# JeongsooP/RGB-no-more

Hardware: AMD Instinct MI355X
Metric: images/sec JPEG-Ti DCT 512x512 train step (higher is better)
Workload: dtype bf16

## Files before the change

include/rgbnm.h:

```cpp
#ifndef RGBNM_H
#define RGBNM_H
#include <stddef.h>
#include <stdint.h>

#ifdef __cplusplus
extern "C" {
#endif

#define RGBNM_ABI_VERSION 3
#define RGBNM_DT_F32 0
#define RGBNM_DT_BF16 1
#define RGBNM_DT_F16 2
#define RGBNM_DT_I16 2

#define RGBNM_EPI_NONE 0
#define RGBNM_EPI_RES 1
#define RGBNM_EPI_GELU 2
#define RGBNM_EPI_POS 3
#define RGBNM_EPI_DGELU 4
#define RGBNM_EPI_TANH 5
#define RGBNM_EPI_DTANH 6
#define RGBNM_EPI_RES_DROP 7
#define RGBNM_EPI_GELU_DROP 8

int rgbnm_abi_version(void);
int rgbnm_set_option(const char* name, int value);
int rgbnm_get_option(const char* name);
int rgbnm_trace_collect(int tag, double* ms_total, double* flops_total, double* bytes_total, int* count);
int rgbnm_trace_reserve(int n_events);
const char* rgbnm_strerror(int code);

int rgbnm_gemm_nt(int dtype, int epi, const void* A, int lda, const void* W, int ldw, void* C, int ldc,
                  const float* bias, const void* R, int ldr, void* C2, int ldc2, const float* pos, int pos_period,
                  int M, int N, int K, int c_f32, void* stream);

int rgbnm_gemm_nt_drop(int dtype, int epi, const void* A, int lda, const void* W, int ldw, void* C, int ldc,
                       const float* bias, const void* R, int ldr, void* C2, int ldc2, const float* pos, int pos_period,
                       int M, int N, int K, int c_f32, const void* seed, float p, int site, int block, void* stream);
int rgbnm_dropout_apply(int dtype, const void* seed, float p, int site, int block, const void* x, int ldx, void* y, int ldy,
                        int M, int N, void* stream);

size_t rgbnm_gemm_tn_workspace(int M, int No, int Ki);
size_t rgbnm_gemm_tn_workspace_splits(int No, int Ki, int splits);
int rgbnm_gemm_tn(int dtype, const void* dY, int ldy, const void* X, int ldx, float* dW, float* db, int M, int No,
                  int Ki, int perm_heads, int accumulate, void* workspace, size_t workspace_bytes, void* stream);

void rgbnm_gemm_tn_group_begin(void);
int rgbnm_gemm_tn_group_end(void* stream);
void rgbnm_gemm_tn_group_begin_n(int max_jobs);
void rgbnm_gemm_tn_group_begin_id(int max_jobs, unsigned long long id);
void rgbnm_gemm_tn_group_abort(unsigned long long id);

typedef struct rgbnm_linear_desc {
  long long w_off;
  long long b_off;
  long long ws_off;
  long long wst_off;
  long long bperm_off;
  int N, K;
  int perm_heads;
  int add_identity;
  int ldn;
  int pair;
  int chain_kind;
  long long chain_off;
  int bias_mode;
  int _pad2;
  long long b2_off;
} rgbnm_linear_desc;

int rgbnm_prep_weights(int dtype, const rgbnm_linear_desc* descs_dev, int ndesc, const float* master, void* shadow,
                       float* bias_perm, void* stream);
int rgbnm_prep_weights_chain(int dtype, const rgbnm_linear_desc* descs_dev, int ndesc, const float* master, void* shadow,
                             float* bias_perm, void* chain_fwd, void* chain_bwd, int skip_chain_shadows, void* stream);

int rgbnm_layernorm_fwd(int dtype, const void* x, const float* gamma, const float* beta, void* y, float* mean,
                        float* rstd, int M, int E, float eps, void* stream);
size_t rgbnm_layernorm_bwd_workspace(int M, int E);
int rgbnm_layernorm_bwd(int dtype, const void* dy, const void* x, const float* gamma, const float* mean,
                        const float* rstd, const void* dres, void* dx, float* dgamma, float* dbeta, int M, int E,
                        int accumulate, void* workspace, size_t workspace_bytes, void* stream);
int rgbnm_head_pool_fwd(int dtype, const void* x, const float* gamma, const float* beta, void* pooled, float* mean,
                        float* rstd, int B, int N, int E, float eps, void* stream);
int rgbnm_head_pool_bwd(int dtype, const void* dpooled, const void* x, const float* gamma, const float* mean,
                        const float* rstd, void* dx, float* dgamma, float* dbeta, int B, int N, int E, int accumulate,
                        void* workspace, size_t workspace_bytes, void* stream);

int rgbnm_attention_fwd(int dtype, const void* qkv, void* out, float* lse, int B, int N, int heads, float scale,
                        void* stream);
int rgbnm_attention_bwd(int dtype, const void* qkv, const void* out, const void* dout, const float* lse, void* dqkv,
                        int B, int N, int heads, float scale, void* stream);

int rgbnm_subblock_embed(int in_dtype, int out_dtype, const void* y, const void* cbcr, const float* conv16,
                         void* feat, int B, int Hb, int Wb, int transpose_a, void* stream);
int rgbnm_subblock_embed_mix(int in_dtype, int out_dtype, const void* y, const void* cbcr, const float* lam_dev, const float* conv16,
                             void* feat, int B, int Hb, int Wb, int transpose_a, void* stream);

#define RGBNM_OP_IDENTITY 0
#define RGBNM_OP_AUTOCONTRAST 1
#define RGBNM_OP_POSTERIZE 2
#define RGBNM_OP_SOLARIZEADD 3
#define RGBNM_OP_COLOR 4
#define RGBNM_OP_CONTRAST 5
#define RGBNM_OP_BRIGHTNESS 6
#define RGBNM_OP_MIDFREQAUG 7
#define RGBNM_OP_CUTOUT 8
#define RGBNM_OP_TRANSLATEX 9
#define RGBNM_OP_TRANSLATEY 10
#define RGBNM_OP_ROTATE90 11
#define RGBNM_OP_AUTOSATURATION 12
#define RGBNM_OP_GRAYSCALE 13
#define RGBNM_OP_CHROMADROP 14
#define RGBNM_OP_SHARPNESS 15
#define RGBNM_OP_INVERT 16
#define RGBNM_OP_SOLARIZE 17
#define RGBNM_OP_FREQENHANCE 18
#define RGBNM_OP_EQUALIZE 19

typedef struct rgbnm_aug_params {
  int crop_i, crop_j, crop_h, crop_w;
  int flip;
  int op[2];
  float fmag[2];
  int iarg0[2], iarg1[2], iarg2[2];
} rgbnm_aug_params;

size_t rgbnm_dct_augment_workspace(int B);
int rgbnm_dct_augment(const int16_t* Yq, const int16_t* CbCrq, const int16_t* quant, const rgbnm_aug_params* params_dev,
                      const rgbnm_aug_params* params_host, const float* conv16, const float* filters, void* outY,
                      void* outC, int out_dtype, int B, int Hy, int Wy, int Hc, int Wc, int entry_clamp, int nops,
                      void* workspace, size_t workspace_bytes, void* stream);
size_t rgbnm_dct_augment_workspace_ex(int B, int size);
int rgbnm_dct_augment_ex(const int16_t* Yq, const int16_t* CbCrq, const int16_t* quant, const rgbnm_aug_params* params_dev,
                         const rgbnm_aug_params* params_host, const float* conv16, const float* filters, void* outY,
                         void* outC, int out_dtype, int size, int B, int Hy, int Wy, int Hc, int Wc, int entry_clamp,
                         int nops, void* workspace, size_t workspace_bytes, void* stream);

int rgbnm_dct_augment_packed(const int16_t* Ypacked, const int16_t* Cpacked, const long long* y_off, const long long* c_off,
                             const int16_t* quant, const rgbnm_aug_params* params_dev, const rgbnm_aug_params* params_host,
                             const float* conv16, const float* filters, void* outY, void* outC, int out_dtype, int size, int B,
                             int Hy, int Wy, int Hc, int Wc, int entry_clamp, int nops, void* workspace, size_t workspace_bytes,
                             void* stream);

int rgbnm_softxent(int dl_dtype, const float* logits, const float* soft_target, const long long* hard_target,
                   float* loss_rows, float* loss, void* dlogits, int B, int C, float grad_scale, void* stream);
int rgbnm_softxent_loss(const float* logits, const float* soft_target, const long long* hard_target, float* loss_rows,
                        float* row_stats, float* loss, unsigned* ticket, int B, int C, void* stream);
int rgbnm_softxent_grad(int dl_dtype, const float* logits, const float* soft_target, const long long* hard_target,
                        const float* row_stats, const float* gout_dev, void* dlogits, int B, int C, float grad_scale, void* stream);
int rgbnm_softxent_loss_mix(const float* logits, const long long* labels, const float* mix_lam_dev, float* loss_rows,
                            float* row_stats, float* loss, unsigned* ticket, int B, int C, void* stream);
int rgbnm_softxent_grad_mix(int dl_dtype, const float* logits, const long long* labels, const float* mix_lam_dev,
                            const float* row_stats, const float* gout_dev, void* dlogits, int B, int C, float grad_scale,
                            void* stream);
int rgbnm_mixup(int in_dtype, int out_dtype, const void* in, void* out, const float* lam_dev, int B,
                long long per_sample, void* stream);
int rgbnm_mixup_target(const long long* labels, float* target, const float* lam_dev, int B, int C, void* stream);
size_t rgbnm_clip_adamw_wd_workspace(void);
int rgbnm_clip_adamw_wd_step(float* p, const float* g, float* m, float* v, const unsigned char* wd_flag_per_256,
                             long long n, float lr, float beta1, float beta2, float eps, int step, float wd_factor,
                             float max_norm, float* norm_out, void* workspace, size_t workspace_bytes, void* stream);

typedef struct rgbnm_vit_cfg {
  int dtype, B, N, E, heads;
  float ln_eps, attn_scale;
} rgbnm_vit_cfg;

typedef struct rgbnm_block_params {
  const float *ln1_g, *ln1_b, *ln2_g, *ln2_b;
  const float *bqkv_perm, *bproj, *b1, *b2;
  const void *wqkv, *wqkv_t, *wproj, *wproj_t, *w1, *w1_t, *w2, *w2_t;
} rgbnm_block_params;

typedef struct rgbnm_block_acts {
  void* x_in;
  void* xn1;
  float *mean1, *rstd1;
  void* qkv;
  float* lse;
  void* attn;
  void* x_mid;
  void* xn2;
  float *mean2, *rstd2;
  void* u;
  void* gl;
  void* x_out;
} rgbnm_block_acts;

typedef struct rgbnm_block_grads {
  float *dln1_g, *dln1_b, *dln2_g, *dln2_b;
  float *dwqkv, *dbqkv, *dwproj, *dbproj, *dw1, *db1, *dw2, *db2;
} rgbnm_block_grads;

typedef struct rgbnm_block_scratch {
  void* du;
  void* dxn;
  void* dx_mid;
  void* dattn;
  void* dqkv;
  void* ws;
  size_t ws_bytes;
} rgbnm_block_scratch;

size_t rgbnm_vit_workspace(const rgbnm_vit_cfg* cfg);
size_t rgbnm_vit_workspace_ex(const rgbnm_vit_cfg* cfg, int n_classes);
int rgbnm_vit_block_fwd(const rgbnm_vit_cfg* cfg, const rgbnm_block_params* p, const rgbnm_block_acts* a,
                        void* stream);
int rgbnm_vit_ln_chain(const rgbnm_vit_cfg* cfg);
int rgbnm_vit_block_fwd_chain(const rgbnm_vit_cfg* cfg, const rgbnm_block_params* p, const rgbnm_block_acts* a,
                              int flags, const rgbnm_block_params* next_p, const rgbnm_block_acts* next_a,
                              void* stream);
int rgbnm_vit_block_bwd(const rgbnm_vit_cfg* cfg, const rgbnm_block_params* p, const rgbnm_block_acts* a,
                        const rgbnm_block_grads* g, const rgbnm_block_scratch* s, const void* dy, void* dx,
                        void* stream);

typedef struct rgbnm_dropout {
  const void* seed;
  float p;
  int block;
  void *dy_m, *dxmid_m;
} rgbnm_dropout;
int rgbnm_vit_block_fwd_drop(const rgbnm_vit_cfg* cfg, const rgbnm_block_params* p, const rgbnm_block_acts* a,
                             const rgbnm_dropout* d, void* stream);
int rgbnm_vit_block_bwd_drop(const rgbnm_vit_cfg* cfg, const rgbnm_block_params* p, const rgbnm_block_acts* a,
                             const rgbnm_block_grads* g, const rgbnm_block_scratch* s, const rgbnm_dropout* d, const void* dy,
                             void* dx, void* stream);

typedef struct rgbnm_chain_block {
  const void* wimg;
  const float *ln1_g, *ln1_b, *ln2_g, *ln2_b, *bqkv_perm, *bproj, *b1, *b2;
  void* xn1; float *mean1, *rstd1;
  void* qkv; float* lse; void* attn; void* x_mid; void* xn2; float *mean2, *rstd2;
  void* u; void* gl; void* x_out;
} rgbnm_chain_block;
size_t rgbnm_chain_block_bytes(void);
long long rgbnm_chain_image_elems(void);
int rgbnm_chain_gather(const void* src, const int* idx, void* dst, long long n, void* stream);
int rgbnm_vit_chain_fwd(const rgbnm_vit_cfg* cfg, const rgbnm_chain_block* blocks, int depth, const void* x0, void* stream);

typedef struct rgbnm_chain_bwd_block {
  const void* wimg;
  const float *ln1_g, *ln2_g;
  const void* x_in; const float *mean1, *rstd1;
  const void* qkv; const float* lse; const void* attn; const void* x_mid; const float *mean2, *rstd2; const void* u;
  const void* dy;
  void* du; void* dx_mid; void* dqkv; void* dx;
  float *part2, *part1;
} rgbnm_chain_bwd_block;
size_t rgbnm_chain_bwd_block_bytes(void);
int rgbnm_vit_chain_bwd(const rgbnm_vit_cfg* cfg, const rgbnm_chain_bwd_block* blocks, int depth, void* dattn, void* stream);
int rgbnm_vit_block_bwd_dw(const rgbnm_vit_cfg* cfg, const rgbnm_block_acts* a, const rgbnm_block_grads* g,
                           const rgbnm_block_scratch* s, const void* dy, const float* part2, const float* part1, void* stream);
int rgbnm_vit_blocks_bwd_dw(const rgbnm_vit_cfg* cfg, int n, const rgbnm_block_acts* const* a, const rgbnm_block_grads* const* g,
                            const rgbnm_block_scratch* const* s, const void* const* dy, const float* const* part2,
                            const float* const* part1, void* stream);
int rgbnm_vit_blocks_bwd_dw_pe(const rgbnm_vit_cfg* cfg, int n, const rgbnm_block_acts* const* a, const rgbnm_block_grads* const* g,
                               const rgbnm_block_scratch* const* s, const void* const* dy, const float* const* part2,
                               const float* const* part1, const void* pe_dx0, const void* pe_feat, float* pe_dw, float* pe_db,
                               void* pe_ws, size_t pe_ws_bytes, void* stream);

int rgbnm_gelu_table_init(void* stream);
int rgbnm_gelu_table_info(int* win16, unsigned* full65536);

int rgbnm_reduce_hold_begin(void);
int rgbnm_reduce_hold_end(void* table, void* table_host, size_t table_bytes, void* stream);
void rgbnm_reduce_hold_cancel(void);
size_t rgbnm_reduce_hold_table_bytes(void);

int rgbnm_patch_embed_fwd(const rgbnm_vit_cfg* cfg, int in_dtype, const void* y, const void* cbcr,
                          const float* conv16, const void* wpe, const float* bpe, const float* pos, void* feat,
                          void* x0, int Hb, int Wb, void* stream);
int rgbnm_patch_embed_fwd_mix(const rgbnm_vit_cfg* cfg, int in_dtype, const void* y, const void* cbcr, const float* lam_dev,
                              const float* conv16, const void* wpe, const float* bpe, const float* pos, void* feat, void* x0,
                              int Hb, int Wb, void* stream);
int rgbnm_patch_embed_bwd(const rgbnm_vit_cfg* cfg, const void* dx0, const void* feat, float* dwpe, float* dbpe,
                          void* ws, size_t ws_bytes, void* stream);

typedef struct rgbnm_head_params {
  const float *ln_g, *ln_b, *b1, *b2;
  const void *w1, *w1_t, *w2, *w2_t;
  int n_classes;
  int _pad;
} rgbnm_head_params;
typedef struct rgbnm_head_acts {
  void* x;
  float *mean, *rstd;
  void* pooled;
  void* h1;
  float* logits;
} rgbnm_head_acts;
typedef struct rgbnm_head_grads {
  float *dln_g, *dln_b, *dw1, *db1, *dw2, *db2;
} rgbnm_head_grads;
int rgbnm_head_fwd(const rgbnm_vit_cfg* cfg, const rgbnm_head_params* p, const rgbnm_head_acts* a, void* stream);
size_t rgbnm_head_bwd_workspace(const rgbnm_vit_cfg* cfg, int n_classes);
int rgbnm_head_bwd(const rgbnm_vit_cfg* cfg, const rgbnm_head_params* p, const rgbnm_head_acts* a,
                   const rgbnm_head_grads* g, const void* dlogits, void* da, void* dpooled, void* dx, void* ws,
                   size_t ws_bytes, void* stream);

int rgbnm_swin_embed(int in_dtype, int out_dtype, const void* y, const void* cbcr, const float* convY, const float* convC,
                     void* feat, int B, int Hb, int Wb, void* stream);
int rgbnm_ln_generic_fwd(int dtype, const void* x, const float* gamma, const float* beta, const void* res,
                         const float* sample_scale, int rows_per_sample, void* y, float* mean, float* rstd, int M, int E,
                         float eps, void* stream);
size_t rgbnm_ln_generic_bwd_workspace(int M, int E);
int rgbnm_ln_generic_bwd(int dtype, const void* dy, const void* x, const float* gamma, const float* mean,
                         const float* rstd, const float* sample_scale, int rows_per_sample, void* dx, float* dgamma,
                         float* dbeta, int M, int E, int accumulate, void* workspace, size_t workspace_bytes,
                         void* stream);
int rgbnm_window_attention_fwd(int dtype, const void* qkv, const float* bias, const float* scale, void* out, float* lse,
                               int B, int res, int C, int heads, int shift, void* stream);
size_t rgbnm_window_attention_bwd_workspace(int B, int res, int heads);
int rgbnm_window_attention_bwd(int dtype, const void* qkv, const void* out, const void* dout, const float* bias,
                               float* dscale , const float* scale, const float* lse, void* dqkv,
                               float* dbias, float* dscale_part, int B, int res, int C, int heads, int shift, void* workspace,
                               size_t workspace_bytes, void* stream);
typedef struct rgbnm_cpb_block {
  const float *w1, *b1, *w2, *ls;
  float *bias, *scale;
  const float *dbias, *dscale;
  float *dw1, *db1, *dw2, *dls;
  int heads, _pad;
} rgbnm_cpb_block;
size_t rgbnm_swin_cpb_table_elems(int nblocks);
int rgbnm_swin_cpb_fwd(const rgbnm_cpb_block* blocks, int nblocks, const float* coords, const int* index, float* table, void* stream);
int rgbnm_swin_cpb_bwd(const rgbnm_cpb_block* blocks, int nblocks, const float* coords, const int* inv_index, const float* table,
                       float* dtable, void* stream);
int rgbnm_merge_gather(int dtype, const void* in, void* out, int B, int res, int C, int inverse, void* stream);
int rgbnm_token_mean(int dtype, const void* in, void* out, int B, int N, int C, int backward, void* stream);


int rgbnm_calib_mfma_bf16(int workgroups, int iters, float* sink, void* stream);
int rgbnm_calib_stream(const void* src, void* dst, size_t bytes, int mode, int workgroups, void* sink, void* stream);
int rgbnm_calib_vmem_issue(int mode, int workgroups, int waves, void* buf, size_t wave_bytes, int ld,
                           unsigned long long* out, void* stream);
int rgbnm_calib_l2(const void* buf, size_t slice_bytes, int iters, int mode, int workgroups, int waves, void* sink,
                   void* stream);
int rgbnm_calib_pipes(const int* role_dev, int waves, int iters, int workgroups, unsigned long long* out, float* sink,
                      void* stream);

int rgbnm_calib_occupy(const void* buf, size_t slice_bytes, int workgroups, int lds_bytes, long long ticks, int mode,
                       const int* stop, void* sink, void* stream);
int rgbnm_calib_occupy_log(const void* buf, size_t slice_bytes, int workgroups, int lds_bytes, long long ticks, int mode,
                           const int* stop, void* sink, unsigned long long* log, void* stream);

#ifdef __cplusplus
}
#endif
#endif
```

rgb-no-more_amd/csrc/gemm_nt_small.hip:

```cpp
#include "common.h"
#include "internal.h"

namespace {

enum { EPI_NONE = 0, EPI_TANH = 5, EPI_DTANH = 6 };

struct SmallNT {
  const bf16* A; const bf16* W; void* C; const float* bias; const bf16* R;
  int lda, ldw, ldc, ldr;
  int M, N, K, c_f32, ntiles;
};

constexpr int RP = 36;

template <int EPI>
__global__ __launch_bounds__(256) void gemm_nt_small_kernel(SmallNT p) {
  __shared__ __attribute__((aligned(16))) float red[4][32 * RP];
  const int tid = threadIdx.x, lane = tid & 63;
  const int w = __builtin_amdgcn_readfirstlane(tid >> 6);
  const int l31 = lane & 31, g = lane >> 5;
  const int m0 = (blockIdx.x / p.ntiles) * 32, n0 = (blockIdx.x % p.ntiles) * 32;
  const bf16* arow = p.A + (size_t)min(m0 + l31, p.M - 1) * p.lda;
  const bf16* wrow = p.W + (size_t)min(n0 + l31, p.N - 1) * p.ldw;
  const int ksteps = (p.K + 15) / 16;
  const int per = (ksteps + 3) / 4;
  const int s0 = w * per, s1 = min(s0 + per, ksteps);
  f32x16 acc;
#pragma unroll
  for (int r = 0; r < 16; ++r) acc[r] = 0.f;
  const bf16x8 zero = {0, 0, 0, 0, 0, 0, 0, 0};
  auto frag = [&](const bf16* row, int s) -> bf16x8 {
    const int k = 16 * s + 8 * g;
    return k < p.K ? *reinterpret_cast<const bf16x8*>(row + k) : zero;
  };
  for (int s = s0; s < s1; s += 4) {
    Frag<bf16> fa[4], fw[4];
#pragma unroll
    for (int u = 0; u < 4; ++u) {
      const int su = s + u < s1 ? s + u : s1 - 1;
      fa[u].v = frag(arow, su);
      fw[u].v = frag(wrow, su);
    }
#pragma unroll
    for (int u = 0; u < 4; ++u)
      if (s + u < s1) mma(acc, fw[u], fa[u]);
  }
#pragma unroll
  for (int q = 0; q < 4; ++q) {
    const f32x4 v = {acc[4 * q + 0], acc[4 * q + 1], acc[4 * q + 2], acc[4 * q + 3]};
    *reinterpret_cast<f32x4*>(&red[w][l31 * RP + 8 * q + 4 * g]) = v;
  }
  __syncthreads();
  const int row = tid >> 3, f0 = (tid & 7) * 4;
  const int gm = m0 + row, gn = n0 + f0;
  if (gm >= p.M || gn >= p.N) return;
  f32x4 v = *reinterpret_cast<const f32x4*>(&red[0][row * RP + f0]);
#pragma unroll
  for (int k = 1; k < 4; ++k) v += *reinterpret_cast<const f32x4*>(&red[k][row * RP + f0]);
  if (p.bias) v += *reinterpret_cast<const f32x4*>(p.bias + gn);
  if (p.c_f32) {
#pragma unroll
    for (int e = 0; e < 4; ++e) {
      if (EPI == EPI_TANH) v[e] = tanhf(v[e]);
      if (EPI == EPI_DTANH) {
        const float h = (float)p.R[(size_t)gm * p.ldr + gn + e];
        v[e] *= (1.f - h * h);
      }
    }
    *reinterpret_cast<f32x4*>(reinterpret_cast<float*>(p.C) + (size_t)gm * p.ldc + gn) = v;
    return;
  }
  bf16x4 o;
#pragma unroll
  for (int e = 0; e < 4; ++e) {
    float x = (float)(bf16)v[e];
    if (EPI == EPI_TANH) x = tanhf(x);
    if (EPI == EPI_DTANH) {
      const float h = (float)p.R[(size_t)gm * p.ldr + gn + e];
      x *= (1.f - h * h);
    }
    o[e] = (bf16)x;
  }
  *reinterpret_cast<bf16x4*>(reinterpret_cast<bf16*>(p.C) + (size_t)gm * p.ldc + gn) = o;
}

}

int rgbnm_launch_nt_small(int epi, const void* A, int lda, const void* W, int ldw, void* C, int ldc, const float* bias,
                          const void* R, int ldr, int c_f32, int M, int N, int K, hipStream_t st) {
  if (M > 512 || K % 8 || N % 4 || lda % 8 || ldw % 8 || ldc % 4 || (epi != EPI_NONE && epi != EPI_TANH && epi != EPI_DTANH))
    return 1;
  if (epi == EPI_DTANH && !R) return RGBNM_EINVAL;
  SmallNT p;
  p.A = (const bf16*)A; p.W = (const bf16*)W; p.C = C; p.bias = bias; p.R = (const bf16*)R;
  p.lda = lda; p.ldw = ldw; p.ldc = ldc; p.ldr = ldr; p.M = M; p.N = N; p.K = K; p.c_f32 = c_f32;
  p.ntiles = cdiv(N, 32);
  const int grid = cdiv(M, 32) * p.ntiles;
  const double mn = (double)M * N;
  const int slot = rgbnm_trace_begin(TR_NT, 2.0 * mn * K, ((double)M * K + (double)N * K) * 2.0 + mn * (c_f32 ? 4.0 : 2.0) +
                                                              (epi == EPI_DTANH ? mn * 2.0 : 0.0), st);
  switch (epi) {
    case EPI_NONE: hipLaunchKernelGGL(gemm_nt_small_kernel<EPI_NONE>, dim3(grid), dim3(256), 0, st, p); break;
    case EPI_TANH: hipLaunchKernelGGL(gemm_nt_small_kernel<EPI_TANH>, dim3(grid), dim3(256), 0, st, p); break;
    default: hipLaunchKernelGGL(gemm_nt_small_kernel<EPI_DTANH>, dim3(grid), dim3(256), 0, st, p); break;
  }
  rgbnm_trace_end(slot, st);
  LAUNCH_CHECK();
  return RGBNM_OK;
}
```

rgb-no-more_amd/csrc/internal.h:

```cpp
#pragma once
#include <hip/hip_runtime.h>

constexpr int RGBNM_TN_MAX_SPLIT = 128;
struct RgbnmTnJob {
  const void* dY; const void* X; float* part; float* bpart;
  int ldy, ldx, M, No, Ki;
  float* dW; float* db; int perm_heads, accumulate;
  int smax;
};
int rgbnm_launch_tn_pipe_group(const RgbnmTnJob* jobs, int n, int* S_out, hipStream_t st, int* direct_out = nullptr);
void rgbnm_tn_defer_begin();
void rgbnm_tn_defer_begin_n(int max_jobs);
int rgbnm_tn_defer_flush(hipStream_t st);
int rgbnm_launch_tn_pipe(const void* dY, int ldy, const void* X, int ldx, float* part, float* bpart, int M, int No,
                         int Ki, int* S_out, hipStream_t st, int smax = 0);

int rgbnm_launch_attn2_fwd(const void* qkv, void* out, float* lse, int B, int N, int heads, float scale,
                           hipStream_t st);
int rgbnm_launch_attn2_bwd(const void* qkv, const void* out, const void* dout, const float* lse, void* dqkv, int B,
                           int N, int heads, float scale, hipStream_t st);

enum { TR_NT = 1, TR_TN = 2, TR_ATTN_FWD = 3, TR_ATTN_BWD = 4, TR_CHAIN_FWD = 5, TR_CHAIN_BWD = 6, TR_AUG = 7, TR_EMBED = 8, TR_OPT = 9 };
int rgbnm_launch_nt_wres(int epi, const void* A, int lda, const void* W, int ldw, void* C, int ldc, const float* bias,
                         const void* R, int ldr, void* C2, int ldc2, int M, int N, int K, hipStream_t st);
int rgbnm_launch_nt_kpipe(int epi, const void* A, int lda, const void* W, int ldw, void* C, int ldc, const float* bias,
                          const void* R, int ldr, void* C2, int ldc2, int M, int N, int K, hipStream_t st);
int rgbnm_launch_nt_kpipe_res_ln(const void* A, int lda, const void* W, int ldw, const float* bias, const void* R,
                                 int ldr, void* x, int ldc, const float* gamma, const float* beta, void* y, int ldy,
                                 float* mean, float* rstd, float eps, int M, int N, int K, hipStream_t st);
int rgbnm_launch_mlp_fwd(const void* X, int ldx, const void* W1, const float* b1, const void* W2, const float* b2,
                         const void* R, int ldr, void* G, void* GP, int ldg, void* Y, int ldy, const float* gamma,
                         const float* beta, void* Y2, int ldy2, float* mean, float* rstd, float eps, int M, int E, int H,
                         hipStream_t st);
int rgbnm_launch_nt_small(int epi, const void* A, int lda, const void* W, int ldw, void* C, int ldc, const float* bias,
                          const void* R, int ldr, int c_f32, int M, int N, int K, hipStream_t st);
int rgbnm_launch_mlp_bwd(const void* DY, int lddy, const void* W2T, const void* W1T, const void* GP, int ldg, void* DU, int ldu,
                         const void* X, int ldx, const float* gamma, const float* mean, const float* rstd, void* DX, int lddx,
                         float* part, int* npanels_out, int M, int E, int H, hipStream_t st);
int rgbnm_launch_nt_kpipe_lnbwd(const void* A, int lda, const void* W, int ldw, const void* X, int ldx,
                                const float* gamma, const float* mean, const float* rstd, const void* dres, int ldr,
                                void* dx, int ldc, float* part, int* npanels_out, int M, int N, int K, hipStream_t st);
struct RgbnmReduceJob {
  const float* part; long long stride; float* out;
  int n, S, cols, perm_heads, accumulate, epw;
};
bool rgbnm_reduce_defer_active();
void rgbnm_reduce_defer_begin();
int rgbnm_reduce_defer_flush(hipStream_t st);
int rgbnm_reduce_submit(const RgbnmReduceJob& job, hipStream_t st);
int rgbnm_trace_begin(int tag, double flops, double bytes, hipStream_t st);
void rgbnm_trace_end(int slot, hipStream_t st);
```

rgb-no-more_amd/csrc/reduce.hip:

```cpp
#include <cstddef>
#include <cstring>
#include "common.h"
#include "internal.h"

namespace {

constexpr int MAXJOBS = 16;
struct Jobs {
  RgbnmReduceJob j[MAXJOBS];
};

thread_local bool g_defer = false;
thread_local int g_njobs = 0;
thread_local Jobs g_jobs;

__device__ __forceinline__ int qkv_row_r(int n, int heads) {
  const int inner = heads * 64;
  const int s3 = n / inner, rem = n % inner;
  return (rem / 64) * 192 + (rem % 64) * 3 + s3;
}

__global__ __launch_bounds__(256) void reduce_multi_kernel(Jobs J) {
  const RgbnmReduceJob jb = J.j[blockIdx.y];
  __shared__ float red[256];
  const int epw = jb.epw, nsg = 256 / epw;
  const int el = threadIdx.x % epw, sg = threadIdx.x / epw;
  for (int base = blockIdx.x * epw; base < jb.n; base += gridDim.x * epw) {
    const int i = base + el;
    float a = 0.f;
    if (i < jb.n) {
      const float* src = jb.part + i;
#pragma unroll 8
      for (int s = sg; s < jb.S; s += nsg) a += src[(size_t)s * jb.stride];
    }
    red[sg * epw + el] = a;
    __syncthreads();
    if (sg == 0 && i < jb.n) {
      float t;
      if (nsg == 4) {
        t = (red[el] + red[epw + el]) + (red[2 * epw + el] + red[3 * epw + el]);
      } else {
        t = 0.f;
        for (int g = 0; g < nsg; ++g) t += red[g * epw + el];
      }
      int o = i;
      if (jb.perm_heads > 0) {
        const int r = i / jb.cols, c = i % jb.cols;
        o = qkv_row_r(r, jb.perm_heads) * jb.cols + c;
      }
      jb.out[o] = jb.accumulate ? (jb.out[o] + t) : t;
    }
    __syncthreads();
  }
}

constexpr int MAXHELD = 384;
struct HeldTable {
  int njobs, total;
  int first[MAXHELD + 1];
  unsigned char vec[MAXHELD];
  RgbnmReduceJob j[MAXHELD];
};
thread_local bool g_hold = false;
thread_local HeldTable g_held;

template <int VEC>
__device__ __forceinline__ void reduce_job(const RgbnmReduceJob& jb, int bx, int nbx, float* red) {
  const int epw = jb.epw, nsg = 256 / epw;
  const int el = threadIdx.x % epw, sg = threadIdx.x / epw;
  for (int base = bx * epw * VEC; base < jb.n; base += nbx * epw * VEC) {
    const int i = base + el * VEC;
    float a[VEC];
#pragma unroll
    for (int v = 0; v < VEC; ++v) a[v] = 0.f;
    if (i < jb.n) {
      const float* src = jb.part + i;
#pragma unroll 8
      for (int s = sg; s < jb.S; s += nsg) {
        if (VEC == 4) {
          const f32x4 q = *reinterpret_cast<const f32x4*>(src + (size_t)s * jb.stride);
#pragma unroll
          for (int v = 0; v < VEC; ++v) a[v] += q[v];
        } else {
          a[0] += src[(size_t)s * jb.stride];
        }
      }
    }
#pragma unroll
    for (int v = 0; v < VEC; ++v) red[(sg * epw + el) * VEC + v] = a[v];
    __syncthreads();
    if (sg == 0 && i < jb.n) {
#pragma unroll
      for (int v = 0; v < VEC; ++v) {
        float t;
        if (nsg == 4) {
          t = (red[el * VEC + v] + red[(epw + el) * VEC + v]) + (red[(2 * epw + el) * VEC + v] + red[(3 * epw + el) * VEC + v]);
        } else {
          t = 0.f;
          for (int g = 0; g < nsg; ++g) t += red[(g * epw + el) * VEC + v];
        }
        int o = i + v;
        if (jb.perm_heads > 0) {
          const int r = o / jb.cols, c = o % jb.cols;
          o = qkv_row_r(r, jb.perm_heads) * jb.cols + c;
        }
        jb.out[o] = jb.accumulate ? (jb.out[o] + t) : t;
      }
    }
    __syncthreads();
  }
}

__global__ __launch_bounds__(256) void reduce_table_kernel(const HeldTable* __restrict__ T) {
  __shared__ __attribute__((aligned(16))) float red[256 * 4];
  int lo = 0, hi = T->njobs - 1;
  while (lo < hi) {
    const int mid = (lo + hi + 1) >> 1;
    if (T->first[mid] <= (int)blockIdx.x) lo = mid;
    else hi = mid - 1;
  }
  const RgbnmReduceJob jb = T->j[lo];
  const int bx = blockIdx.x - T->first[lo], nbx = T->first[lo + 1] - T->first[lo];
  if (T->vec[lo]) reduce_job<4>(jb, bx, nbx, red);
  else reduce_job<1>(jb, bx, nbx, red);
}

int launch(const Jobs& J, int njobs, hipStream_t st) {
  int gx = 1;
  for (int k = 0; k < njobs; ++k) {
    const int need = cdiv(J.j[k].n, J.j[k].epw);
    gx = need > gx ? need : gx;
  }
  if (gx > 1024) gx = 1024;
  hipLaunchKernelGGL(reduce_multi_kernel, dim3(gx, njobs), dim3(256), 0, st, J);
  LAUNCH_CHECK();
  return RGBNM_OK;
}

}

bool rgbnm_reduce_defer_active() { return g_defer; }
void rgbnm_reduce_defer_begin() {
  g_defer = true;
  g_njobs = 0;
}

int rgbnm_reduce_defer_flush(hipStream_t st) {
  g_defer = false;
  const int n = g_njobs;
  g_njobs = 0;
  return n > 0 ? launch(g_jobs, n, st) : RGBNM_OK;
}

int rgbnm_reduce_submit(const RgbnmReduceJob& job, hipStream_t st) {
  if (job.n <= 0 || job.S <= 0 || (job.epw != 64 && job.epw != 8)) return RGBNM_EINVAL;
  if (g_hold && g_held.njobs < MAXHELD) {
    g_held.j[g_held.njobs++] = job;
    return RGBNM_OK;
  }
  if (g_defer) {
    if (g_njobs == MAXJOBS) {
      const int rc = launch(g_jobs, g_njobs, st);
      if (rc != RGBNM_OK) return rc;
      g_njobs = 0;
    }
    g_jobs.j[g_njobs++] = job;
    return RGBNM_OK;
  }
  Jobs one;
  one.j[0] = job;
  return launch(one, 1, st);
}

extern "C" {

int rgbnm_reduce_hold_begin(void) {
  if (g_hold) return RGBNM_EINVAL;
  g_hold = true;
  g_held.njobs = 0;
  return RGBNM_OK;
}

void rgbnm_reduce_hold_cancel(void) {
  g_hold = false;
  g_held.njobs = 0;
}

int rgbnm_reduce_hold_end(void* table_dev, void* table_host, size_t table_bytes, void* stream) {
  if (!g_hold) return RGBNM_OK;
  g_hold = false;
  const int n = g_held.njobs;
  if (n == 0) return RGBNM_OK;
  if (!table_dev || !table_host || table_bytes < sizeof(HeldTable)) return RGBNM_EWORKSPACE;
  int total = 0;
  for (int k = 0; k < n; ++k) {
    const RgbnmReduceJob& j = g_held.j[k];
    const bool vec = j.n % 4 == 0 && j.stride % 4 == 0 && ((size_t)j.part & 15) == 0 && (j.perm_heads <= 0 || j.cols % 4 == 0);
    g_held.vec[k] = vec ? 1 : 0;
    g_held.first[k] = total;
    const int need = cdiv(j.n, j.epw * (vec ? 4 : 1));
    total += need > 1024 ? 1024 : need;
  }
  for (int k = n; k <= MAXHELD; ++k) g_held.first[k] = total;
  g_held.total = total;
  hipStream_t st = (hipStream_t)stream;
  const size_t used = offsetof(HeldTable, j) + sizeof(RgbnmReduceJob) * (size_t)n;
  if (memcmp(table_host, &g_held, used) != 0) {
    hipStreamCaptureStatus cap = hipStreamCaptureStatusNone;
    if (hipStreamIsCapturing(st, &cap) != hipSuccess) { g_held.njobs = 0; return RGBNM_ELAUNCH; }
    if (cap != hipStreamCaptureStatusNone) {
      memcpy(table_host, &g_held, used);
      if (hipMemcpyAsync(table_dev, table_host, used, hipMemcpyHostToDevice, st) != hipSuccess) {
        (void)hipGetLastError();
        memset(table_host, 0, used);
        g_held.njobs = 0;
        return RGBNM_EINVAL;
      }
    } else {
      if (hipMemcpyAsync(table_dev, &g_held, used, hipMemcpyHostToDevice, st) != hipSuccess) {
        g_held.njobs = 0;
        return RGBNM_ELAUNCH;
      }
      memcpy(table_host, &g_held, used);
    }
  }
  g_held.njobs = 0;
  hipLaunchKernelGGL(reduce_table_kernel, dim3(total), dim3(256), 0, st, (const HeldTable*)table_dev);
  LAUNCH_CHECK();
  return RGBNM_OK;
}

size_t rgbnm_reduce_hold_table_bytes(void) { return sizeof(HeldTable); }

}
```

rgb-no-more_amd/csrc/vit.hip:

```cpp
#include "common.h"
#include "../../include/rgbnm.h"

#define TRY(x)                 \
  do {                         \
    int rc__ = (x);            \
    if (rc__ != 0) return rc__; \
  } while (0)

static inline size_t max_sz(size_t a, size_t b) { return a > b ? a : b; }

#include <string.h>
#include <atomic>
#include <mutex>
#include <vector>
#include "internal.h"
namespace {
std::mutex g_trace_mu;
struct TraceRec { hipEvent_t a, b; int tag; double flops, bytes; };
std::vector<TraceRec> g_recs;
std::vector<hipEvent_t> g_event_pool;
hipEvent_t take_event() {
  if (!g_event_pool.empty()) { hipEvent_t e = g_event_pool.back(); g_event_pool.pop_back(); return e; }
  hipEvent_t e = nullptr;
  if (hipEventCreate(&e) != hipSuccess) return nullptr;
  return e;
}
struct Opt { const char* name; std::atomic<int> value; };
Opt g_opts[] = {{"nt_staged", 1}, {"tn_tr", 1}, {"tn_pipe", 1}, {"attn_v2", 1}, {"nt_wres", 1}, {"nt_kpipe", 1}, {"attn_persist", 1}, {"ln_fuse", 1}, {"tn_group", 2}, {"trace", 0}, {"tn_wgs", 512}, {"mlp_fuse", 1}, {"nt_cold", 0}, {"mlp_bwd", 1}, {"nt_small", 1}, {"mlp_dmast", 1}, {"gelu_table", 1}, {"ln_rows", 1}, {"kp8", 1}, {"win_xcd", 1}, {"kp_persist", 1}, {"fwd_chain", 1}, {"bwd_chain", 1}, {"tn_direct", 1}, {"tn_pack", 1}, {"tn_wide", 1}};
}

int rgbnm_trace_begin(int tag, double flops, double bytes, hipStream_t st) {
  int mask = 0;
  for (auto& o : g_opts) if (!strcmp(o.name, "trace")) mask = o.value.load(std::memory_order_relaxed);
  if (!((mask >> tag) & 1)) return -1;
  std::lock_guard<std::mutex> lk(g_trace_mu);
  TraceRec r;
  r.a = take_event();
  r.b = take_event();
  if (!r.a || !r.b) return -1;
  r.tag = tag; r.flops = flops; r.bytes = bytes;
  (void)hipEventRecord(r.a, st);
  g_recs.push_back(r);
  return (int)g_recs.size() - 1;
}
void rgbnm_trace_end(int slot, hipStream_t st) {
  if (slot < 0) return;
  std::lock_guard<std::mutex> lk(g_trace_mu);
  if (slot >= 0 && slot < (int)g_recs.size()) (void)hipEventRecord(g_recs[slot].b, st);
}

extern "C" {

int rgbnm_abi_version(void) { return RGBNM_ABI_VERSION; }

int rgbnm_set_option(const char* name, int value) {
  for (auto& o : g_opts)
    if (name && !strcmp(o.name, name)) { o.value.store(value, std::memory_order_relaxed); return RGBNM_OK; }
  return RGBNM_EINVAL;
}
int rgbnm_get_option(const char* name) {
  for (auto& o : g_opts)
    if (name && !strcmp(o.name, name)) return o.value.load(std::memory_order_relaxed);
  return -1;
}

int rgbnm_trace_reserve(int n_events) {
  if (n_events < 0 || n_events > (1 << 16)) return RGBNM_EINVAL;
  std::lock_guard<std::mutex> lk(g_trace_mu);
  while ((int)g_event_pool.size() < n_events) {
    hipEvent_t e = nullptr;
    if (hipEventCreate(&e) != hipSuccess) return RGBNM_ELAUNCH;
    g_event_pool.push_back(e);
  }
  return RGBNM_OK;
}

int rgbnm_trace_collect(int tag, double* ms_total, double* flops_total, double* bytes_total, int* count) {
  double ms = 0, fl = 0, by = 0;
  int n = 0;
  std::lock_guard<std::mutex> lk(g_trace_mu);
  std::vector<TraceRec> keep;
  for (auto& r : g_recs) {
    if (r.tag != tag) { keep.push_back(r); continue; }
    if (hipEventSynchronize(r.b) != hipSuccess) return RGBNM_ELAUNCH;
    float t = 0.f;
    if (hipEventElapsedTime(&t, r.a, r.b) != hipSuccess) return RGBNM_ELAUNCH;
    ms += t; fl += r.flops; by += r.bytes; ++n;
    g_event_pool.push_back(r.a);
    g_event_pool.push_back(r.b);
  }
  g_recs.swap(keep);
  if (ms_total) *ms_total = ms;
  if (flops_total) *flops_total = fl;
  if (bytes_total) *bytes_total = by;
  if (count) *count = n;
  return RGBNM_OK;
}

const char* rgbnm_strerror(int code) {
  switch (code) {
    case 0: return "ok";
    case RGBNM_EINVAL: return "invalid argument (null pointer, bad shape, alignment or dtype)";
    case RGBNM_ELAUNCH: return "HIP kernel launch failed";
    case RGBNM_EWORKSPACE: return "workspace too small";
    default: return "unknown rgbnm error";
  }
}

static bool fused_dx_lnbwd(int dt, const void* A, int lda, const void* Wt, int ldw, const void* x, const float* gamma,
                           const float* mean, const float* rstd, const void* dres, void* dx, float* dgamma,
                           float* dbeta, int M, int E, int K, void* ws, size_t ws_bytes, hipStream_t st) {
  if (dt != RGBNM_DT_BF16 || E != 192 || !rgbnm_get_option("ln_fuse") || !rgbnm_get_option("nt_kpipe")) return false;
  if (ws_bytes < (size_t)cdiv(M, cdiv(M, 512)) * 2 * E * sizeof(float)) return false;
  int npanels = 0;
  const int rc = rgbnm_launch_nt_kpipe_lnbwd(A, lda, Wt, ldw, x, E, gamma, mean, rstd, dres, E, dx, E, (float*)ws,
                                             &npanels, M, E, K, st);
  if (rc != RGBNM_OK) return false;
  RgbnmReduceJob j;
  j.part = (const float*)ws; j.stride = 2LL * E; j.out = dgamma; j.n = E; j.S = npanels; j.cols = 1; j.perm_heads = 0;
  j.accumulate = 0; j.epw = 8;
  if (rgbnm_reduce_submit(j, st) != RGBNM_OK) return false;
  j.part = (const float*)ws + E; j.out = dbeta;
  return rgbnm_reduce_submit(j, st) == RGBNM_OK;
}

static bool fused_mlp_bwd(int dt, const void* dy, const void* w2t, const void* w1t, const void* gp, void* du, const void* x,
                          const float* gamma, const float* mean, const float* rstd, void* dx, float* dgamma, float* dbeta,
                          int M, int E, void* ws, size_t ws_bytes, hipStream_t st) {
  if (dt != RGBNM_DT_BF16 || E != 192 || !rgbnm_get_option("mlp_bwd") || !rgbnm_get_option("ln_fuse")) return false;
  if (ws_bytes < (size_t)cdiv(M, cdiv(M, 256)) * 2 * E * sizeof(float)) return false;
  int npanels = 0;
  const int rc = rgbnm_launch_mlp_bwd(dy, E, w2t, w1t, gp, 4 * E, du, 4 * E, x, E, gamma, mean, rstd, dx, E, (float*)ws,
                                      &npanels, M, E, 4 * E, st);
  if (rc != RGBNM_OK) return false;
  RgbnmReduceJob j;
  j.part = (const float*)ws; j.stride = 2LL * E; j.out = dgamma; j.n = E; j.S = npanels; j.cols = 1; j.perm_heads = 0;
  j.accumulate = 0; j.epw = 8;
  if (rgbnm_reduce_submit(j, st) != RGBNM_OK) return false;
  j.part = (const float*)ws + E; j.out = dbeta;
  return rgbnm_reduce_submit(j, st) == RGBNM_OK;
}

static size_t block_ws_offsets(int M, int E, int I, size_t (&off)[7]) {
  const size_t sz[6] = {rgbnm_gemm_tn_workspace(M, E, 4 * E), rgbnm_gemm_tn_workspace(M, 4 * E, E),
                        rgbnm_gemm_tn_workspace(M, E, I),     rgbnm_gemm_tn_workspace(M, 3 * I, E),
                        rgbnm_layernorm_bwd_workspace(M, E),  rgbnm_layernorm_bwd_workspace(M, E)};
  off[0] = 0;
  for (int i = 0; i < 6; ++i) off[i + 1] = off[i] + ((sz[i] + 255) & ~(size_t)255);
  return off[6];
}

size_t rgbnm_vit_workspace(const rgbnm_vit_cfg* c) { return rgbnm_vit_workspace_ex(c, 1024); }

size_t rgbnm_vit_workspace_ex(const rgbnm_vit_cfg* c, int n_classes) {
  if (!c) return 0;
  if (n_classes < 1024) n_classes = 1024;
  const int M = c->B * c->N, E = c->E, I = c->heads * 64;
  size_t off[7];
  size_t w = block_ws_offsets(M, E, I, off);
  w = max_sz(w, rgbnm_gemm_tn_workspace(M, E, 384));
  w = max_sz(w, rgbnm_gemm_tn_workspace(c->B, n_classes, E));
  w = max_sz(w, rgbnm_layernorm_bwd_workspace(M, E));
  w = max_sz(w, (size_t)c->B * 2 * E * sizeof(float));
  return w;
}

int rgbnm_vit_ln_chain(const rgbnm_vit_cfg* c) {
  if (!c) return 0;
  return c->dtype == RGBNM_DT_BF16 && c->E == 192 && c->B * c->N >= 8192 && rgbnm_get_option("ln_fuse") &&
         rgbnm_get_option("nt_kpipe");
}

int rgbnm_vit_block_fwd_chain(const rgbnm_vit_cfg* c, const rgbnm_block_params* p, const rgbnm_block_acts* a, int flags,
                              const rgbnm_block_params* next_p, const rgbnm_block_acts* next_a, void* st) {
  if (!c || !p || !a) return RGBNM_EINVAL;
  const int dt = c->dtype, M = c->B * c->N, E = c->E, I = c->heads * 64;
  const bool chain = rgbnm_vit_ln_chain(c) != 0;
  if ((flags & 1) && !chain) return RGBNM_EINVAL;
  if (!(flags & 1))
    TRY(rgbnm_layernorm_fwd(dt, a->x_in, p->ln1_g, p->ln1_b, a->xn1, a->mean1, a->rstd1, M, E, c->ln_eps, st));
  TRY(rgbnm_gemm_nt(dt, RGBNM_EPI_NONE, a->xn1, E, p->wqkv, E, a->qkv, 3 * I, p->bqkv_perm, 0, 0, 0, 0, 0, 0, M,
                    3 * I, E, 0, st));
  TRY(rgbnm_attention_fwd(dt, a->qkv, a->attn, a->lse, c->B, c->N, c->heads, c->attn_scale, st));
  if (!chain || rgbnm_launch_nt_kpipe_res_ln(a->attn, I, p->wproj, I, p->bproj, a->x_in, E, a->x_mid, E, p->ln2_g,
                                             p->ln2_b, a->xn2, E, a->mean2, a->rstd2, c->ln_eps, M, E, I,
                                             (hipStream_t)st) != RGBNM_OK) {
    TRY(rgbnm_gemm_nt(dt, RGBNM_EPI_RES, a->attn, I, p->wproj, I, a->x_mid, E, p->bproj, a->x_in, E, 0, 0, 0, 0, M, E,
                      I, 0, st));
    TRY(rgbnm_layernorm_fwd(dt, a->x_mid, p->ln2_g, p->ln2_b, a->xn2, a->mean2, a->rstd2, M, E, c->ln_eps, st));
  }
  const bool to_next = chain && next_p && next_a;
  if (to_next && next_a->x_in != a->x_out) return RGBNM_EINVAL;
  if (dt == RGBNM_DT_BF16 && rgbnm_get_option("mlp_fuse")) {
    const int rc = rgbnm_launch_mlp_fwd(a->xn2, E, p->w1, p->b1, p->w2, p->b2, a->x_mid, E, a->gl, a->u, 4 * E, a->x_out, E,
                                        to_next ? next_p->ln1_g : nullptr, to_next ? next_p->ln1_b : nullptr,
                                        to_next ? next_a->xn1 : nullptr, E, to_next ? next_a->mean1 : nullptr,
                                        to_next ? next_a->rstd1 : nullptr, c->ln_eps, M, E, 4 * E, (hipStream_t)st);
    if (rc <= 0) return rc;
  }
  TRY(rgbnm_gemm_nt(dt, RGBNM_EPI_GELU, a->xn2, E, p->w1, E, a->gl, 4 * E, p->b1, 0, 0, a->u, 4 * E, 0, 0, M, 4 * E,
                    E, 0, st));
  if (to_next) {
    const int rc = rgbnm_launch_nt_kpipe_res_ln(a->gl, 4 * E, p->w2, 4 * E, p->b2, a->x_mid, E, a->x_out, E,
                                                next_p->ln1_g, next_p->ln1_b, next_a->xn1, E, next_a->mean1,
                                                next_a->rstd1, c->ln_eps, M, E, 4 * E, (hipStream_t)st);
    if (rc != RGBNM_OK) return rc < 0 ? rc : RGBNM_EINVAL;
    return RGBNM_OK;
  }
  TRY(rgbnm_gemm_nt(dt, RGBNM_EPI_RES, a->gl, 4 * E, p->w2, 4 * E, a->x_out, E, p->b2, a->x_mid, E, 0, 0, 0, 0, M, E,
                    4 * E, 0, st));
  return RGBNM_OK;
}

int rgbnm_vit_block_fwd(const rgbnm_vit_cfg* c, const rgbnm_block_params* p, const rgbnm_block_acts* a, void* st) {
  return rgbnm_vit_block_fwd_chain(c, p, a, 0, nullptr, nullptr, st);
}

int rgbnm_vit_block_fwd_drop(const rgbnm_vit_cfg* c, const rgbnm_block_params* p, const rgbnm_block_acts* a, const rgbnm_dropout* d,
                             void* st) {
  if (!c || !p || !a || !d) return RGBNM_EINVAL;
  const int dt = c->dtype, M = c->B * c->N, E = c->E, I = c->heads * 64;
  TRY(rgbnm_layernorm_fwd(dt, a->x_in, p->ln1_g, p->ln1_b, a->xn1, a->mean1, a->rstd1, M, E, c->ln_eps, st));
  TRY(rgbnm_gemm_nt(dt, RGBNM_EPI_NONE, a->xn1, E, p->wqkv, E, a->qkv, 3 * I, p->bqkv_perm, 0, 0, 0, 0, 0, 0, M,
                    3 * I, E, 0, st));
  TRY(rgbnm_attention_fwd(dt, a->qkv, a->attn, a->lse, c->B, c->N, c->heads, c->attn_scale, st));
  TRY(rgbnm_gemm_nt_drop(dt, RGBNM_EPI_RES_DROP, a->attn, I, p->wproj, I, a->x_mid, E, p->bproj, a->x_in, E, 0, 0, 0, 0, M, E, I,
                         0, d->seed, d->p, 0, d->block, st));
  TRY(rgbnm_layernorm_fwd(dt, a->x_mid, p->ln2_g, p->ln2_b, a->xn2, a->mean2, a->rstd2, M, E, c->ln_eps, st));
  TRY(rgbnm_gemm_nt_drop(dt, RGBNM_EPI_GELU_DROP, a->xn2, E, p->w1, E, a->gl, 4 * E, p->b1, 0, 0, a->u, 4 * E, 0, 0, M, 4 * E, E,
                         0, d->seed, d->p, 1, d->block, st));
  TRY(rgbnm_gemm_nt_drop(dt, RGBNM_EPI_RES_DROP, a->gl, 4 * E, p->w2, 4 * E, a->x_out, E, p->b2, a->x_mid, E, 0, 0, 0, 0, M, E,
                         4 * E, 0, d->seed, d->p, 2, d->block, st));
  return RGBNM_OK;
}

static int block_bwd(const rgbnm_vit_cfg* c, const rgbnm_block_params* p, const rgbnm_block_acts* a, const rgbnm_block_grads* g,
                     const rgbnm_block_scratch* s, const rgbnm_dropout* d, const void* dy, void* dx, void* st) {
  if (!c || !p || !a || !g || !s || !dy || !dx) return RGBNM_EINVAL;
  if (d && (!d->dy_m || !d->dxmid_m || d->dy_m == d->dxmid_m)) return RGBNM_EINVAL;
  const int dt = c->dtype, M = c->B * c->N, E = c->E, I = c->heads * 64;
  size_t off[7];
  if (s->ws_bytes < block_ws_offsets(M, E, I, off)) return RGBNM_EWORKSPACE;
  char* wsb = (char*)s->ws;
#define WS(i) (wsb + off[i]), (off[(i) + 1] - off[i])
  rgbnm_reduce_defer_begin();
  bool tn_open = false;
  const int rc = [&]() -> int {
  int group = rgbnm_get_option("tn_group");
  const bool wide4 = rgbnm_get_option("tn_wide") && E % 384 == 0 && I % 384 == 0 && M % 64 == 0;
  if (group == 2 && E > 192 && !wide4) group = 1;
  if (group) { rgbnm_tn_defer_begin(); tn_open = true; }
  const void* dyg = dy;
  if (d) {
    TRY(rgbnm_dropout_apply(dt, d->seed, d->p, 2, d->block, dy, E, d->dy_m, E, M, E, st));
    dyg = d->dy_m;
  }
  TRY(rgbnm_gemm_tn(dt, dyg, E, a->gl, 4 * E, g->dw2, g->db2, M, E, 4 * E, 0, 0, WS(0), st));
  const bool mlp_bwd_fused = !d && fused_mlp_bwd(dt, dy, p->w2_t, p->w1_t, a->u, s->du, a->x_mid, p->ln2_g, a->mean2, a->rstd2,
                                                 s->dx_mid, g->dln2_g, g->dln2_b, M, E, WS(4), (hipStream_t)st);
  if (!mlp_bwd_fused)
    TRY(rgbnm_gemm_nt(dt, RGBNM_EPI_DGELU, dyg, E, p->w2_t, E, s->du, 4 * E, 0, a->u, 4 * E, 0, 0, 0, 0, M, 4 * E, E, 0,
                      st));
  TRY(rgbnm_gemm_tn(dt, s->du, 4 * E, a->xn2, E, g->dw1, g->db1, M, 4 * E, E, 0, 0, WS(1), st));
  if (group == 1) { tn_open = false; TRY(rgbnm_tn_defer_flush((hipStream_t)st)); }
  if (mlp_bwd_fused) {
  } else if (!fused_dx_lnbwd(dt, s->du, 4 * E, p->w1_t, 4 * E, a->x_mid, p->ln2_g, a->mean2, a->rstd2, dy, s->dx_mid,
                      g->dln2_g, g->dln2_b, M, E, 4 * E, WS(4), (hipStream_t)st)) {
    TRY(rgbnm_gemm_nt(dt, RGBNM_EPI_NONE, s->du, 4 * E, p->w1_t, 4 * E, s->dxn, E, 0, 0, 0, 0, 0, 0, 0, M, E, 4 * E,
                      0, st));
    TRY(rgbnm_layernorm_bwd(dt, s->dxn, a->x_mid, p->ln2_g, a->mean2, a->rstd2, dy, s->dx_mid, g->dln2_g, g->dln2_b,
                            M, E, 0, WS(4), st));
  }
  const void* dxmg = s->dx_mid;
  if (d) {
    TRY(rgbnm_dropout_apply(dt, d->seed, d->p, 0, d->block, s->dx_mid, E, d->dxmid_m, E, M, E, st));
    dxmg = d->dxmid_m;
  }
  if (group == 1) { rgbnm_tn_defer_begin(); tn_open = true; }
  TRY(rgbnm_gemm_tn(dt, dxmg, E, a->attn, I, g->dwproj, g->dbproj, M, E, I, 0, 0, WS(2), st));
  TRY(rgbnm_gemm_nt(dt, RGBNM_EPI_NONE, dxmg, E, p->wproj_t, E, s->dattn, I, 0, 0, 0, 0, 0, 0, 0, M, I, E, 0, st));
  TRY(rgbnm_attention_bwd(dt, a->qkv, a->attn, s->dattn, a->lse, s->dqkv, c->B, c->N, c->heads, c->attn_scale, st));
  TRY(rgbnm_gemm_tn(dt, s->dqkv, 3 * I, a->xn1, E, g->dwqkv, g->dbqkv, M, 3 * I, E, c->heads, 0, WS(3), st));
  if (group) { tn_open = false; TRY(rgbnm_tn_defer_flush((hipStream_t)st)); }
  if (!fused_dx_lnbwd(dt, s->dqkv, 3 * I, p->wqkv_t, 3 * I, a->x_in, p->ln1_g, a->mean1, a->rstd1, s->dx_mid, dx,
                      g->dln1_g, g->dln1_b, M, E, 3 * I, WS(5), (hipStream_t)st)) {
    TRY(rgbnm_gemm_nt(dt, RGBNM_EPI_NONE, s->dqkv, 3 * I, p->wqkv_t, 3 * I, s->dxn, E, 0, 0, 0, 0, 0, 0, 0, M, E,
                      3 * I, 0, st));
    TRY(rgbnm_layernorm_bwd(dt, s->dxn, a->x_in, p->ln1_g, a->mean1, a->rstd1, s->dx_mid, dx, g->dln1_g, g->dln1_b, M,
                            E, 0, WS(5), st));
  }
  return RGBNM_OK;
  }();
#undef WS
  const int rt = tn_open ? rgbnm_tn_defer_flush((hipStream_t)st) : RGBNM_OK;
  const int rf = rgbnm_reduce_defer_flush((hipStream_t)st);
  return rc != RGBNM_OK ? rc : (rt != RGBNM_OK ? rt : rf);
}

int rgbnm_vit_block_bwd(const rgbnm_vit_cfg* c, const rgbnm_block_params* p, const rgbnm_block_acts* a,
                        const rgbnm_block_grads* g, const rgbnm_block_scratch* s, const void* dy, void* dx, void* st) {
  return block_bwd(c, p, a, g, s, nullptr, dy, dx, st);
}

int rgbnm_vit_block_bwd_drop(const rgbnm_vit_cfg* c, const rgbnm_block_params* p, const rgbnm_block_acts* a,
                             const rgbnm_block_grads* g, const rgbnm_block_scratch* s, const rgbnm_dropout* d, const void* dy,
                             void* dx, void* st) {
  if (!d) return RGBNM_EINVAL;
  return block_bwd(c, p, a, g, s, d, dy, dx, st);
}

int rgbnm_vit_blocks_bwd_dw(const rgbnm_vit_cfg* c, int n, const rgbnm_block_acts* const* a, const rgbnm_block_grads* const* g,
                            const rgbnm_block_scratch* const* s, const void* const* dy, const float* const* part2,
                            const float* const* part1, void* st) {
  return rgbnm_vit_blocks_bwd_dw_pe(c, n, a, g, s, dy, part2, part1, nullptr, nullptr, nullptr, nullptr, nullptr, 0, st);
}

int rgbnm_vit_blocks_bwd_dw_pe(const rgbnm_vit_cfg* c, int n, const rgbnm_block_acts* const* a, const rgbnm_block_grads* const* g,
                               const rgbnm_block_scratch* const* s, const void* const* dy, const float* const* part2,
                               const float* const* part1, const void* pe_dx0, const void* pe_feat, float* pe_dw, float* pe_db,
                               void* pe_ws, size_t pe_ws_bytes, void* st) {
  if (!c || n < 1 || n > 12 || !a || !g || !s || !dy || !part2 || !part1) return RGBNM_EINVAL;
  if (pe_dx0 && (!pe_feat || !pe_dw || !pe_ws)) return RGBNM_EINVAL;
  const int dt = c->dtype, M = c->B * c->N, E = c->E, I = c->heads * 64;
  size_t off[7];
  const size_t need = block_ws_offsets(M, E, I, off);
  for (int i = 0; i < n; ++i) {
    if (!a[i] || !g[i] || !s[i] || !dy[i] || !part2[i] || !part1[i]) return RGBNM_EINVAL;
    if (s[i]->ws_bytes < need) return RGBNM_EWORKSPACE;
    for (int k = 0; k < i; ++k)
      if (s[k]->ws == s[i]->ws) return RGBNM_EINVAL;
  }
  rgbnm_reduce_defer_begin();
  bool tn_open = false;
  const int rc = [&]() -> int {
    const int group = rgbnm_get_option("tn_group");
    if (group) { rgbnm_tn_defer_begin_n(group == 1 ? 2 : 4 * n + (pe_dx0 ? 1 : 0)); tn_open = true; }
    for (int i = 0; i < n; ++i) {
      char* wsb = (char*)s[i]->ws;
#define WS(k) (wsb + off[k]), (off[(k) + 1] - off[k])
      TRY(rgbnm_gemm_tn(dt, dy[i], E, a[i]->gl, 4 * E, g[i]->dw2, g[i]->db2, M, E, 4 * E, 0, 0, WS(0), st));
      TRY(rgbnm_gemm_tn(dt, s[i]->du, 4 * E, a[i]->xn2, E, g[i]->dw1, g[i]->db1, M, 4 * E, E, 0, 0, WS(1), st));
      TRY(rgbnm_gemm_tn(dt, s[i]->dx_mid, E, a[i]->attn, I, g[i]->dwproj, g[i]->dbproj, M, E, I, 0, 0, WS(2), st));
      TRY(rgbnm_gemm_tn(dt, s[i]->dqkv, 3 * I, a[i]->xn1, E, g[i]->dwqkv, g[i]->dbqkv, M, 3 * I, E, c->heads, 0, WS(3), st));
#undef WS
    }
    if (pe_dx0) TRY(rgbnm_gemm_tn(dt, pe_dx0, E, pe_feat, 384, pe_dw, pe_db, M, E, 384, 0, 0, pe_ws, pe_ws_bytes, st));
    if (group) { tn_open = false; TRY(rgbnm_tn_defer_flush((hipStream_t)st)); }
    for (int i = 0; i < n; ++i) {
      RgbnmReduceJob j;
      j.stride = 2LL * E; j.n = E; j.S = c->B; j.cols = 1; j.perm_heads = 0; j.accumulate = 0; j.epw = 8;
      j.part = part2[i]; j.out = g[i]->dln2_g;
      TRY(rgbnm_reduce_submit(j, (hipStream_t)st));
      j.part = part2[i] + E; j.out = g[i]->dln2_b;
      TRY(rgbnm_reduce_submit(j, (hipStream_t)st));
      j.part = part1[i]; j.out = g[i]->dln1_g;
      TRY(rgbnm_reduce_submit(j, (hipStream_t)st));
      j.part = part1[i] + E; j.out = g[i]->dln1_b;
      TRY(rgbnm_reduce_submit(j, (hipStream_t)st));
    }
    return RGBNM_OK;
  }();
  const int rt = tn_open ? rgbnm_tn_defer_flush((hipStream_t)st) : RGBNM_OK;
  const int rf = rgbnm_reduce_defer_flush((hipStream_t)st);
  return rc != RGBNM_OK ? rc : (rt != RGBNM_OK ? rt : rf);
}

int rgbnm_vit_block_bwd_dw(const rgbnm_vit_cfg* c, const rgbnm_block_acts* a, const rgbnm_block_grads* g,
                           const rgbnm_block_scratch* s, const void* dy, const float* part2, const float* part1, void* st) {
  return rgbnm_vit_blocks_bwd_dw(c, 1, &a, &g, &s, &dy, &part2, &part1, st);
}

int rgbnm_patch_embed_fwd_mix(const rgbnm_vit_cfg* c, int in_dtype, const void* y, const void* cbcr, const float* lam_dev,
                              const float* conv16, const void* wpe, const float* bpe, const float* pos, void* feat, void* x0, int Hb,
                              int Wb, void* st) {
  if (!c) return RGBNM_EINVAL;
  const int M = c->B * c->N;
  if ((Hb / 2) * (Wb / 2) != c->N) return RGBNM_EINVAL;
  TRY(rgbnm_subblock_embed_mix(in_dtype, c->dtype, y, cbcr, lam_dev, conv16, feat, c->B, Hb, Wb, 0, st));
  TRY(rgbnm_gemm_nt(c->dtype, RGBNM_EPI_POS, feat, 384, wpe, 384, x0, c->E, bpe, 0, 0, 0, 0, pos, c->N, M, c->E, 384,
                    0, st));
  return RGBNM_OK;
}

int rgbnm_patch_embed_fwd(const rgbnm_vit_cfg* c, int in_dtype, const void* y, const void* cbcr, const float* conv16,
                          const void* wpe, const float* bpe, const float* pos, void* feat, void* x0, int Hb, int Wb,
                          void* st) {
  return rgbnm_patch_embed_fwd_mix(c, in_dtype, y, cbcr, nullptr, conv16, wpe, bpe, pos, feat, x0, Hb, Wb, st);
}

int rgbnm_patch_embed_bwd(const rgbnm_vit_cfg* c, const void* dx0, const void* feat, float* dwpe, float* dbpe,
                          void* ws, size_t ws_bytes, void* st) {
  if (!c) return RGBNM_EINVAL;
  return rgbnm_gemm_tn(c->dtype, dx0, c->E, feat, 384, dwpe, dbpe, c->B * c->N, c->E, 384, 0, 0, ws, ws_bytes, st);
}

int rgbnm_head_fwd(const rgbnm_vit_cfg* c, const rgbnm_head_params* p, const rgbnm_head_acts* a, void* st) {
  if (!c || !p || !a) return RGBNM_EINVAL;
  const int dt = c->dtype, E = c->E, C = p->n_classes;
  TRY(rgbnm_head_pool_fwd(dt, a->x, p->ln_g, p->ln_b, a->pooled, a->mean, a->rstd, c->B, c->N, E, c->ln_eps, st));
  TRY(rgbnm_gemm_nt(dt, RGBNM_EPI_TANH, a->pooled, E, p->w1, E, a->h1, E, p->b1, 0, 0, 0, 0, 0, 0, c->B, E, E, 0, st));
  TRY(rgbnm_gemm_nt(dt, RGBNM_EPI_NONE, a->h1, E, p->w2, E, a->logits, C, p->b2, 0, 0, 0, 0, 0, 0, c->B, C, E, 1, st));
  return RGBNM_OK;
}

size_t rgbnm_head_bwd_workspace(const rgbnm_vit_cfg* c, int n_classes) {
  if (!c) return 0;
  return ((rgbnm_gemm_tn_workspace(c->B, n_classes, c->E) + 255) & ~(size_t)255) + ((rgbnm_gemm_tn_workspace(c->B, c->E, c->E) + 255) & ~(size_t)255) +
         (size_t)c->B * 2 * c->E * sizeof(float);
}

int rgbnm_head_bwd(const rgbnm_vit_cfg* c, const rgbnm_head_params* p, const rgbnm_head_acts* a,
                   const rgbnm_head_grads* g, const void* dlogits, void* da, void* dpooled, void* dx, void* ws,
                   size_t ws_bytes, void* st) {
  if (!c || !p || !a || !g || !dlogits || !da || !dpooled || !dx) return RGBNM_EINVAL;
  const int dt = c->dtype, E = c->E, C = p->n_classes, B = c->B;
  const size_t s1 = (rgbnm_gemm_tn_workspace(B, C, E) + 255) & ~(size_t)255, s2 = (rgbnm_gemm_tn_workspace(B, E, E) + 255) & ~(size_t)255;
  const size_t s3 = (size_t)B * 2 * E * sizeof(float);
  const bool apart = ws_bytes >= s1 + s2 + s3;
  char* w1 = (char*)ws;
  char* w2 = apart ? w1 + s1 : w1;
  char* w3 = apart ? w2 + s2 : w1;
  const size_t b1 = apart ? s1 : ws_bytes, b2 = apart ? s2 : ws_bytes, b3 = apart ? ws_bytes - s1 - s2 : ws_bytes;
  const bool grouped = apart && rgbnm_get_option("tn_group") != 0;
  if (grouped) rgbnm_tn_defer_begin();
  const int rc = [&]() -> int {
    TRY(rgbnm_gemm_tn(dt, dlogits, C, a->h1, E, g->dw2, g->db2, B, C, E, 0, 0, w1, b1, st));
    TRY(rgbnm_gemm_nt(dt, RGBNM_EPI_DTANH, dlogits, C, p->w2_t, C, da, E, 0, a->h1, E, 0, 0, 0, 0, B, E, C, 0, st));
    TRY(rgbnm_gemm_tn(dt, da, E, a->pooled, E, g->dw1, g->db1, B, E, E, 0, 0, w2, b2, st));
    return RGBNM_OK;
  }();
  const int rt = grouped ? rgbnm_tn_defer_flush((hipStream_t)st) : RGBNM_OK;
  if (rc != RGBNM_OK) return rc;
  if (rt != RGBNM_OK) return rt;
  TRY(rgbnm_gemm_nt(dt, RGBNM_EPI_NONE, da, E, p->w1_t, E, dpooled, E, 0, 0, 0, 0, 0, 0, 0, B, E, E, 0, st));
  TRY(rgbnm_head_pool_bwd(dt, dpooled, a->x, p->ln_g, a->mean, a->rstd, dx, g->dln_g, g->dln_b, B, c->N, E, 0, w3, b3, st));
  return RGBNM_OK;
}

}
```

rgb-no-more_amd/lib.py:

```python
import ctypes as C
import os

import torch

HERE = os.path.dirname(os.path.abspath(__file__))
LIB_PATH = os.path.join(HERE, "librgbnm.so")

DT_F32, DT_BF16, DT_F16 = 0, 1, 2
EPI_NONE, EPI_RES, EPI_GELU, EPI_POS, EPI_DGELU, EPI_TANH, EPI_DTANH = range(7)
EPI_RES_DROP, EPI_GELU_DROP = 7, 8

_vp, _i, _f, _sz, _ll = C.c_void_p, C.c_int, C.c_float, C.c_size_t, C.c_longlong
HOST_WAIT = {"sec": 0.0}


class LinearDesc(C.Structure):
    _fields_ = [("w_off", _ll), ("b_off", _ll), ("ws_off", _ll), ("wst_off", _ll), ("bperm_off", _ll),
                ("N", _i), ("K", _i), ("perm_heads", _i), ("add_identity", _i), ("ldn", _i), ("pair", _i),
                ("chain_kind", _i), ("chain_off", _ll), ("bias_mode", _i), ("_pad2", _i), ("b2_off", _ll)]


class VitCfg(C.Structure):
    _fields_ = [("dtype", _i), ("B", _i), ("N", _i), ("E", _i), ("heads", _i), ("ln_eps", _f), ("attn_scale", _f)]


class BlockParams(C.Structure):
    _fields_ = [(n, _vp) for n in ("ln1_g", "ln1_b", "ln2_g", "ln2_b", "bqkv_perm", "bproj", "b1", "b2",
                                   "wqkv", "wqkv_t", "wproj", "wproj_t", "w1", "w1_t", "w2", "w2_t")]


class BlockActs(C.Structure):
    _fields_ = [(n, _vp) for n in ("x_in", "xn1", "mean1", "rstd1", "qkv", "lse", "attn", "x_mid", "xn2", "mean2",
                                   "rstd2", "u", "gl", "x_out")]


class BlockGrads(C.Structure):
    _fields_ = [(n, _vp) for n in ("dln1_g", "dln1_b", "dln2_g", "dln2_b", "dwqkv", "dbqkv", "dwproj", "dbproj",
                                   "dw1", "db1", "dw2", "db2")]


class BlockScratch(C.Structure):
    _fields_ = [("du", _vp), ("dxn", _vp), ("dx_mid", _vp), ("dattn", _vp), ("dqkv", _vp), ("ws", _vp),
                ("ws_bytes", _sz)]


class Dropout(C.Structure):
    _fields_ = [("seed", _vp), ("p", _f), ("block", _i), ("dy_m", _vp), ("dxmid_m", _vp)]


class HeadParams(C.Structure):
    _fields_ = [(n, _vp) for n in ("ln_g", "ln_b", "b1", "b2", "w1", "w1_t", "w2", "w2_t")] + \
               [("n_classes", _i), ("_pad", _i)]


class HeadActs(C.Structure):
    _fields_ = [(n, _vp) for n in ("x", "mean", "rstd", "pooled", "h1", "logits")]


class HeadGrads(C.Structure):
    _fields_ = [(n, _vp) for n in ("dln_g", "dln_b", "dw1", "db1", "dw2", "db2")]


class CpbBlock(C.Structure):
    _fields_ = [(n, _vp) for n in ("w1", "b1", "w2", "ls", "bias", "scale", "dbias", "dscale", "dw1", "db1", "dw2", "dls")] + \
               [("heads", _i), ("_pad", _i)]


class ChainBlock(C.Structure):
    _fields_ = [(n, _vp) for n in ("wimg", "ln1_g", "ln1_b", "ln2_g", "ln2_b", "bqkv_perm", "bproj", "b1", "b2", "xn1", "mean1",
                                   "rstd1", "qkv", "lse", "attn", "x_mid", "xn2", "mean2", "rstd2", "u", "gl", "x_out")]


class ChainBwdBlock(C.Structure):
    _fields_ = [(n, _vp) for n in ("wimg", "ln1_g", "ln2_g", "x_in", "mean1", "rstd1", "qkv", "lse", "attn", "x_mid", "mean2",
                                   "rstd2", "u", "dy", "du", "dx_mid", "dqkv", "dx", "part2", "part1")]


ABI_VERSION = 3

_P = C.POINTER
PROTOTYPES = {
    "rgbnm_abi_version": (_i, []),
    "rgbnm_strerror": (C.c_char_p, [_i]),
    "rgbnm_set_option": (_i, [C.c_char_p, _i]),
    "rgbnm_gemm_tn_group_begin": (None, []),
    "rgbnm_gemm_tn_group_begin_n": (None, [_i]),
    "rgbnm_gemm_tn_group_begin_id": (None, [_i, C.c_ulonglong]),
    "rgbnm_gemm_tn_group_abort": (None, [C.c_ulonglong]),
    "rgbnm_gemm_tn_group_end": (_i, [_vp]),
    "rgbnm_get_option": (_i, [C.c_char_p]),
    "rgbnm_trace_collect": (_i, [_i, _vp, _vp, _vp, _vp]),
    "rgbnm_trace_reserve": (_i, [_i]),
    "rgbnm_gemm_nt": (_i, [_i, _i, _vp, _i, _vp, _i, _vp, _i, _vp, _vp, _i, _vp, _i, _vp, _i, _i, _i, _i, _i, _vp]),
    "rgbnm_gemm_nt_drop": (_i, [_i, _i, _vp, _i, _vp, _i, _vp, _i, _vp, _vp, _i, _vp, _i, _vp, _i, _i, _i, _i, _i, _vp, _f, _i,
                                _i, _vp]),
    "rgbnm_dropout_apply": (_i, [_i, _vp, _f, _i, _i, _vp, _i, _vp, _i, _i, _i, _vp]),
    "rgbnm_gemm_tn_workspace": (_sz, [_i, _i, _i]),
    "rgbnm_gemm_tn_workspace_splits": (_sz, [_i, _i, _i]),
    "rgbnm_gemm_tn": (_i, [_i, _vp, _i, _vp, _i, _vp, _vp, _i, _i, _i, _i, _i, _vp, _sz, _vp]),
    "rgbnm_prep_weights": (_i, [_i, _vp, _i, _vp, _vp, _vp, _vp]),
    "rgbnm_prep_weights_chain": (_i, [_i, _vp, _i, _vp, _vp, _vp, _vp, _vp, _i, _vp]),
    "rgbnm_layernorm_fwd": (_i, [_i, _vp, _vp, _vp, _vp, _vp, _vp, _i, _i, _f, _vp]),
    "rgbnm_layernorm_bwd_workspace": (_sz, [_i, _i]),
    "rgbnm_layernorm_bwd": (_i, [_i, _vp, _vp, _vp, _vp, _vp, _vp, _vp, _vp, _vp, _i, _i, _i, _vp, _sz, _vp]),
    "rgbnm_head_pool_fwd": (_i, [_i, _vp, _vp, _vp, _vp, _vp, _vp, _i, _i, _i, _f, _vp]),
    "rgbnm_head_pool_bwd": (_i, [_i, _vp, _vp, _vp, _vp, _vp, _vp, _vp, _vp, _i, _i, _i, _i, _vp, _sz, _vp]),
    "rgbnm_attention_fwd": (_i, [_i, _vp, _vp, _vp, _i, _i, _i, _f, _vp]),
    "rgbnm_attention_bwd": (_i, [_i, _vp, _vp, _vp, _vp, _vp, _i, _i, _i, _f, _vp]),
    "rgbnm_subblock_embed": (_i, [_i, _i, _vp, _vp, _vp, _vp, _i, _i, _i, _i, _vp]),
    "rgbnm_subblock_embed_mix": (_i, [_i, _i, _vp, _vp, _vp, _vp, _vp, _i, _i, _i, _i, _vp]),
    "rgbnm_dct_augment_workspace": (_sz, [_i]),
    "rgbnm_dct_augment": (_i, [_vp, _vp, _vp, _vp, _vp, _vp, _vp, _vp, _vp, _i, _i, _i, _i, _i, _i, _i, _i, _vp, _sz,
                               _vp]),
    "rgbnm_dct_augment_workspace_ex": (_sz, [_i, _i]),
    "rgbnm_dct_augment_ex": (_i, [_vp, _vp, _vp, _vp, _vp, _vp, _vp, _vp, _vp, _i, _i, _i, _i, _i, _i, _i, _i, _i, _vp,
                                  _sz, _vp]),
    "rgbnm_dct_augment_packed": (_i, [_vp, _vp, _vp, _vp, _vp, _vp, _vp, _vp, _vp, _vp, _vp, _i, _i, _i, _i, _i, _i, _i, _i,
                                      _i, _vp, _sz, _vp]),
    "rgbnm_softxent": (_i, [_i, _vp, _vp, _vp, _vp, _vp, _vp, _i, _i, _f, _vp]),
    "rgbnm_softxent_loss": (_i, [_vp, _vp, _vp, _vp, _vp, _vp, _vp, _i, _i, _vp]),
    "rgbnm_softxent_grad": (_i, [_i, _vp, _vp, _vp, _vp, _vp, _vp, _i, _i, _f, _vp]),
    "rgbnm_softxent_loss_mix": (_i, [_vp, _vp, _vp, _vp, _vp, _vp, _vp, _i, _i, _vp]),
    "rgbnm_softxent_grad_mix": (_i, [_i, _vp, _vp, _vp, _vp, _vp, _vp, _i, _i, _f, _vp]),
    "rgbnm_mixup": (_i, [_i, _i, _vp, _vp, _vp, _i, _ll, _vp]),
    "rgbnm_mixup_target": (_i, [_vp, _vp, _vp, _i, _i, _vp]),
    "rgbnm_clip_adamw_wd_workspace": (_sz, []),
    "rgbnm_clip_adamw_wd_step": (_i, [_vp, _vp, _vp, _vp, _vp, _ll, _f, _f, _f, _f, _i, _f, _f, _vp, _vp, _sz, _vp]),
    "rgbnm_vit_workspace": (_sz, [_P(VitCfg)]),
    "rgbnm_vit_workspace_ex": (_sz, [_P(VitCfg), _i]),
    "rgbnm_head_bwd_workspace": (_sz, [_vp, _i]),
    "rgbnm_gelu_table_init": (_i, [_vp]),
    "rgbnm_gelu_table_info": (_i, [_vp, _vp]),
    "rgbnm_reduce_hold_begin": (_i, []),
    "rgbnm_reduce_hold_end": (_i, [_vp, _vp, _sz, _vp]),
    "rgbnm_reduce_hold_cancel": (None, []),
    "rgbnm_reduce_hold_table_bytes": (_sz, []),
    "rgbnm_vit_block_fwd": (_i, [_P(VitCfg), _P(BlockParams), _P(BlockActs), _vp]),
    "rgbnm_vit_ln_chain": (_i, [_P(VitCfg)]),
    "rgbnm_swin_embed": (_i, [_i, _i, _vp, _vp, _vp, _vp, _vp, _i, _i, _i, _vp]),
    "rgbnm_ln_generic_fwd": (_i, [_i, _vp, _vp, _vp, _vp, _vp, _i, _vp, _vp, _vp, _i, _i, _f, _vp]),
    "rgbnm_ln_generic_bwd_workspace": (_sz, [_i, _i]),
    "rgbnm_ln_generic_bwd": (_i, [_i, _vp, _vp, _vp, _vp, _vp, _vp, _i, _vp, _vp, _vp, _i, _i, _i, _vp, _sz, _vp]),
    "rgbnm_window_attention_fwd": (_i, [_i, _vp, _vp, _vp, _vp, _vp, _i, _i, _i, _i, _i, _vp]),
    "rgbnm_window_attention_bwd_workspace": (_sz, [_i, _i, _i]),
    "rgbnm_window_attention_bwd": (_i, [_i, _vp, _vp, _vp, _vp, _vp, _vp, _vp, _vp, _vp, _vp, _i, _i, _i, _i, _i, _vp, _sz, _vp]),
    "rgbnm_swin_cpb_table_elems": (_sz, [_i]),
    "rgbnm_swin_cpb_fwd": (_i, [_vp, _i, _vp, _vp, _vp, _vp]),
    "rgbnm_swin_cpb_bwd": (_i, [_vp, _i, _vp, _vp, _vp, _vp, _vp]),
    "rgbnm_merge_gather": (_i, [_i, _vp, _vp, _i, _i, _i, _i, _vp]),
    "rgbnm_token_mean": (_i, [_i, _vp, _vp, _i, _i, _i, _i, _vp]),
    "rgbnm_calib_mfma_bf16": (_i, [_i, _i, _vp, _vp]),
    "rgbnm_calib_stream": (_i, [_vp, _vp, _sz, _i, _i, _vp, _vp]),
    "rgbnm_calib_vmem_issue": (_i, [_i, _i, _i, _vp, _sz, _i, _vp, _vp]),
    "rgbnm_calib_l2": (_i, [_vp, _sz, _i, _i, _i, _i, _vp, _vp]),
    "rgbnm_calib_pipes": (_i, [_vp, _i, _i, _i, _vp, _vp, _vp]),
    "rgbnm_calib_occupy": (_i, [_vp, _sz, _i, _i, C.c_longlong, _i, _vp, _vp, _vp]),
    "rgbnm_calib_occupy_log": (_i, [_vp, _sz, _i, _i, C.c_longlong, _i, _vp, _vp, _vp, _vp]),
    "rgbnm_chain_block_bytes": (_sz, []),
    "rgbnm_chain_image_elems": (_ll, []),
    "rgbnm_chain_gather": (_i, [_vp, _vp, _vp, _ll, _vp]),
    "rgbnm_vit_chain_fwd": (_i, [_P(VitCfg), _P(ChainBlock), _i, _vp, _vp]),
    "rgbnm_chain_bwd_block_bytes": (_sz, []),
    "rgbnm_vit_chain_bwd": (_i, [_P(VitCfg), _P(ChainBwdBlock), _i, _vp, _vp]),
    "rgbnm_vit_block_bwd_dw": (_i, [_P(VitCfg), _P(BlockActs), _P(BlockGrads), _P(BlockScratch), _vp, _vp, _vp, _vp]),
    "rgbnm_vit_blocks_bwd_dw": (_i, [_P(VitCfg), _i, _vp, _vp, _vp, _vp, _vp, _vp, _vp]),
    "rgbnm_vit_blocks_bwd_dw_pe": (_i, [_P(VitCfg), _i, _vp, _vp, _vp, _vp, _vp, _vp, _vp, _vp, _vp, _vp, _vp, _sz, _vp]),
    "rgbnm_vit_block_fwd_chain": (_i, [_P(VitCfg), _P(BlockParams), _P(BlockActs), _i, _P(BlockParams), _P(BlockActs), _vp]),
    "rgbnm_vit_block_bwd": (_i, [_P(VitCfg), _P(BlockParams), _P(BlockActs), _P(BlockGrads), _P(BlockScratch), _vp,
                                 _vp, _vp]),
    "rgbnm_vit_block_fwd_drop": (_i, [_P(VitCfg), _P(BlockParams), _P(BlockActs), _P(Dropout), _vp]),
    "rgbnm_vit_block_bwd_drop": (_i, [_P(VitCfg), _P(BlockParams), _P(BlockActs), _P(BlockGrads), _P(BlockScratch), _P(Dropout),
                                      _vp, _vp, _vp]),
    "rgbnm_patch_embed_fwd": (_i, [_P(VitCfg), _i, _vp, _vp, _vp, _vp, _vp, _vp, _vp, _vp, _i, _i, _vp]),
    "rgbnm_patch_embed_fwd_mix": (_i, [_P(VitCfg), _i, _vp, _vp, _vp, _vp, _vp, _vp, _vp, _vp, _vp, _i, _i, _vp]),
    "rgbnm_patch_embed_bwd": (_i, [_P(VitCfg), _vp, _vp, _vp, _vp, _vp, _sz, _vp]),
    "rgbnm_head_fwd": (_i, [_P(VitCfg), _P(HeadParams), _P(HeadActs), _vp]),
    "rgbnm_head_bwd": (_i, [_P(VitCfg), _P(HeadParams), _P(HeadActs), _P(HeadGrads), _vp, _vp, _vp, _vp, _vp, _sz,
                            _vp]),
}

_lib = None


class RgbnmError(RuntimeError):
    pass


def lib():
    global _lib
    if _lib is None:
        if not os.path.exists(LIB_PATH):
            raise RgbnmError(f"HIP extension missing: {LIB_PATH} (run `python -c 'import __graft_entry__ as g; g.build()'`). "
                             "There is no CPU fallback.")
        L = C.CDLL(LIB_PATH)
        for name, (res, args) in PROTOTYPES.items():
            fn = getattr(L, name)
            fn.restype = res
            fn.argtypes = args
        if L.rgbnm_abi_version() != ABI_VERSION:
            raise RgbnmError(f"{LIB_PATH} has ABI version {L.rgbnm_abi_version()}, this binding expects {ABI_VERSION}: rebuild "
                             "(python rgb-no-more_amd/build.py)")
        if L.rgbnm_chain_block_bytes() != C.sizeof(ChainBlock) or L.rgbnm_chain_bwd_block_bytes() != C.sizeof(ChainBwdBlock):
            raise RgbnmError("rgbnm_chain_block layout mismatch between librgbnm.so and lib.py")
        _lib = L
    return _lib


def source_hash():
    import hashlib
    h = hashlib.sha256()
    csrc = os.path.join(HERE, "csrc")
    files = sorted(os.path.join(csrc, f) for f in os.listdir(csrc) if f.endswith((".hip", ".inc", ".h", ".c")))
    files.append(os.path.join(os.path.dirname(HERE), "include", "rgbnm.h"))
    for f in files:
        h.update(os.path.basename(f).encode())
        with open(f, "rb") as fh:
            h.update(fh.read())
    return h.hexdigest()[:16]


def check(rc, what=""):
    if rc != 0:
        msg = lib().rgbnm_strerror(rc).decode()
        raise RgbnmError(f"{what}: rgbnm error {rc}: {msg}")


def dt_of(t):
    if t == torch.float32:
        return DT_F32
    if t == torch.bfloat16:
        return DT_BF16
    if t == torch.float16:
        return DT_F16
    raise TypeError(f"unsupported dtype {t} (float32, bfloat16 or float16)")


def ptr(t):
    return None if t is None else t.data_ptr()


_raw_stream = getattr(torch._C, "_cuda_getCurrentRawStream", None)


def stream():
    if _raw_stream is not None:
        return _raw_stream(torch.cuda.current_device())
    return torch.cuda.current_stream().cuda_stream


def require_cuda(*tensors):
    for t in tensors:
        if t is not None and not t.is_cuda:
            raise RgbnmError("rgb-no-more_amd kernels need device (HIP) tensors; there is no CPU fallback")
        if t is not None and not t.is_contiguous():
            raise RgbnmError("tensor must be contiguous")
```

rgb-no-more_amd/plainvit.py:

```python
import ctypes as C
import numpy as np
import math
import threading
import warnings
from collections import OrderedDict

import torch
from torch import nn

from . import dct_ops as dops
from . import lib as L
from .cls_transforms import LazyMixed
from .flatparams import FlatParamModule, align as _align


class ResidualAdd(nn.Module):
    def __init__(self, fn):
        super().__init__()
        self.fn = fn


class MultiHeadAttention(nn.Module):
    def __init__(self, emb_size, num_heads, head_size, input_embed=-1, device="cpu", dtype=torch.float32):
        super().__init__()
        inner = num_heads * head_size
        self.qkv = nn.Linear(emb_size if input_embed < 0 else input_embed, inner * 3, device=device, dtype=dtype)
        self.projection = nn.Linear(inner, emb_size, device=device, dtype=dtype)


class PatchEmbedding_DCT_Group(nn.Module):

    def __init__(self, patch_size=16, emb_size=768, use_subblock=True, chroma_scale=2, device="cpu",
                 dtype=torch.float32):
        super().__init__()
        assert not (patch_size & (patch_size - 1)) and patch_size >= 2, \
            f"Patch size should be 2^n (n>0, n=int). Current value: {patch_size}"
        if patch_size != 16 or chroma_scale != 2 or not use_subblock:
            raise NotImplementedError("HIP path covers patch_size=16, 4:2:0, use_subblock=True (JPEG-Ti/S configs)")
        self.patch_size = patch_size
        fin = patch_size ** 2 + 2 * (patch_size // chroma_scale) ** 2
        self.projection = nn.Sequential(nn.Linear(fin, emb_size, device=device, dtype=dtype))
        self.conv_Y = dops.generate_conversion_matrix(8, patch_size // 8, scale=True, dtype=torch.float32)


class PatchEmbedding_DCT_Separate_subblock(nn.Module):

    def __init__(self, patch_size=16, emb_size=768, chroma_scale=2, device="cpu", dtype=torch.float32):
        super().__init__()
        assert not (patch_size & (patch_size - 1)) and patch_size >= 2, \
            f"Patch size should be 2^n (n>0, n=int). Current value: {patch_size}"
        if patch_size != 16 or chroma_scale != 2:
            raise NotImplementedError("HIP path covers patch_size=16, 4:2:0 (JPEG-Ti/S configs)")
        self.patch_size = patch_size
        kw = dict(device=device, dtype=dtype)
        self.projection_Y = nn.Sequential(nn.Identity(), nn.Linear(256, emb_size // 6 * 4, **kw))
        self.projection_C = nn.Sequential(nn.Identity(), nn.Linear(128, emb_size // 6 * 2, **kw))
        self.linearMix = nn.Linear(emb_size, emb_size, **kw)
        self.conv_Y = dops.generate_conversion_matrix(8, patch_size // 8, scale=True, dtype=torch.float32)


class PatchEmbedding_DCT_Separate(nn.Module):

    def __init__(self, patch_size=16, emb_size=768, chroma_scale=2, device="cpu", dtype=torch.float32):
        super().__init__()
        assert not (patch_size & (patch_size - 1)) and patch_size >= 2, \
            f"Patch size should be 2^n (n>0, n=int). Current value: {patch_size}"
        assert patch_size // chroma_scale >= 8, \
            (f"Patch size for both Y and CbCr should be larger than 8 for this embedding method. Current patch size (Y): "
             f"{patch_size}, chroma scale: {chroma_scale}, patch_size (CbCr): {patch_size // chroma_scale}")
        if patch_size != 16 or chroma_scale != 2:
            raise NotImplementedError("HIP path covers patch_size=16, 4:2:0 (JPEG-Ti/S configs)")
        self.patch_size = patch_size
        kw = dict(device=device, dtype=dtype)
        nb = 6
        self.LinearY = nn.ModuleList([nn.Linear(64, emb_size // nb, **kw) for _ in range(4)])
        self.LinearC = nn.ModuleList([nn.Linear(64, emb_size // nb, **kw) for _ in range(2)])
        self.PreMixActivation = nn.Identity()
        self.LinearMix = nn.Linear((emb_size // nb) * nb, emb_size, **kw)
        self.projection = nn.Sequential(self.PreMixActivation, self.LinearMix)


class PatchEmbedding_DCT_Concat(nn.Module):

    def __init__(self, patch_size=16, emb_size=768, use_subblock=True, device="cpu", dtype=torch.float32):
        super().__init__()
        assert not (patch_size & (patch_size - 1)) and patch_size >= 2, \
            f"Patch size should be 2^n (n>0, n=int). Current value: {patch_size}"
        if patch_size != 16 or not use_subblock:
            raise NotImplementedError("HIP path covers patch_size=16 with sub-block conversion (JPEG-Ti/S configs)")
        self.patch_size = patch_size
        kw = dict(device=device, dtype=dtype)
        self.projectionY = nn.Sequential(nn.Identity(), nn.Linear(patch_size ** 2, emb_size, **kw))
        self.projectionC = nn.Sequential(nn.Identity(), nn.Linear(patch_size ** 2, emb_size, **kw))
        self.convMat = dops.generate_conversion_matrix(8, patch_size // 8, scale=True, dtype=torch.float32)
        self.conv_Y = self.convMat


def sincos_table(h, w, e, device="cpu"):
    hg, wg = torch.meshgrid(torch.arange(h), torch.arange(w), indexing="ij")
    fr = torch.log(torch.tensor(10000, dtype=torch.int32)) / (e // 4 - 1)
    fr = torch.exp(-torch.arange(e // 4, dtype=torch.float32) * fr)
    ph = torch.einsum("p,f->pf", hg.flatten().float(), fr)
    pw = torch.einsum("p,f->pf", wg.flatten().float(), fr)
    return torch.cat((pw.sin(), pw.cos(), ph.sin(), ph.cos()), dim=-1).contiguous().to(device)


CHAIN_MAX_DEPTH = 12


class _Arena:

    def __init__(self, model, B, cdtype, need_grad):
        dev = model._flat.device
        E, I, N, D = model.emb_size, model.inner, model.n_tokens, model.depth
        M = B * N
        T = cdtype
        self.B, self.cdtype, self.need_grad = B, cdtype, need_grad
        e = lambda *s, dt=T: torch.empty(*s, device=dev, dtype=dt)
        f32 = torch.float32
        self.cfg = L.VitCfg(L.dt_of(T), B, N, E, model.num_heads, 1e-5, 1.0 / math.sqrt(E))
        self.feat = e(M, 384)
        if model.embed_kind == "concat":
            self.featC = e(B * 98, 384)
            self.pe_ty, self.pe_tc = e(B * 196, E), e(B * 98, E)
        elif model.embed_kind != "group":
            self.pe_g, self.pe_gp = e(M, E), e(M, E)
            if need_grad:
                self.pe_dh = e(M, E)
        nx = D + 1 if need_grad else 2
        self.x = [e(M, E) for _ in range(nx)]
        nb = D if need_grad else 1
        self.blk = []
        for _ in range(nb):
            self.blk.append(dict(xn1=e(M, E), mean1=e(M, dt=f32), rstd1=e(M, dt=f32), qkv=e(M, 3 * I),
                                 lse=e(B * model.num_heads * N, dt=f32), attn=e(M, I), x_mid=e(M, E), xn2=e(M, E),
                                 mean2=e(M, dt=f32), rstd2=e(M, dt=f32), u=e(M, 4 * E), gl=e(M, 4 * E)))
        self.hmean, self.hrstd = e(M, dt=f32), e(M, dt=f32)
        self.pooled, self.h1 = e(B, E), e(B, E)
        ws_bytes = L.lib().rgbnm_vit_workspace_ex(C.byref(self.cfg), model._ncls_pad)
        self.ws = torch.empty(ws_bytes, device=dev, dtype=torch.uint8)
        if need_grad:
            self.du, self.dxn, self.dx_mid = e(M, 4 * E), e(M, E), e(M, E)
            self.dattn, self.dqkv = e(M, I), e(M, 3 * I)
            self.dx = [e(M, E), e(M, E)]
            self.da, self.dpooled = e(B, E), e(B, E)
            self.scratch = L.BlockScratch(self.du.data_ptr(), self.dxn.data_ptr(), self.dx_mid.data_ptr(),
                                          self.dattn.data_ptr(), self.dqkv.data_ptr(), self.ws.data_ptr(), ws_bytes)
        self.ws_bytes = ws_bytes
        self.ws_blk = self.ws_head = self.hold_table = self.hold_table_host = self.scratch_blk = None
        self.chain_table = None
        self.chain_bwd_table = self.chain_bwd_dy = None
        self.acts = []
        for i in range(D):
            b = self.blk[i if need_grad else 0]
            xi, xo = (self.x[i], self.x[i + 1]) if need_grad else (self.x[i & 1], self.x[(i + 1) & 1])
            self.acts.append(L.BlockActs(xi.data_ptr(), b["xn1"].data_ptr(), b["mean1"].data_ptr(),
                                         b["rstd1"].data_ptr(), b["qkv"].data_ptr(), b["lse"].data_ptr(),
                                         b["attn"].data_ptr(), b["x_mid"].data_ptr(), b["xn2"].data_ptr(),
                                         b["mean2"].data_ptr(), b["rstd2"].data_ptr(), b["u"].data_ptr(),
                                         b["gl"].data_ptr(), xo.data_ptr()))

    def xbuf(self, i):
        return self.x[i] if self.need_grad else self.x[i & 1]


_HOLDER = threading.local()


class _FwdState:

    def __init__(self, model, arena, gbuf):
        self.model, self.arena, self.gbuf = model, arena, gbuf
        self.holding = False
        self.drop = self.drop_seed = None

    def begin_hold(self):
        m, a = self.model, self.arena
        gs = m._grad_sync
        if not m.defer_grad_reduction or (gs is not None and gs.bucket_elems < m._gflat.numel()):
            return
        pe = m.__dict__.get("_pe_params")
        if pe is None:
            pe = m.__dict__["_pe_params"] = [p for n, p in m._named.items() if n.startswith("patchembed.")]
        if not all(p.requires_grad for p in pe):
            return
        if a.ws_blk is None:
            a.ws_blk = torch.empty(m.depth * a.ws_bytes, device=a.ws.device, dtype=torch.uint8)
            a.ws_head = torch.empty(L.lib().rgbnm_head_bwd_workspace(C.byref(a.cfg), m._ncls_pad), device=a.ws.device, dtype=torch.uint8)
            a.hold_table = torch.zeros(L.lib().rgbnm_reduce_hold_table_bytes(), device=a.ws.device, dtype=torch.uint8)
            a.hold_table_host = torch.zeros(a.hold_table.numel(), dtype=torch.uint8)
            a.scratch_blk = [L.BlockScratch(a.du.data_ptr(), a.dxn.data_ptr(), a.dx_mid.data_ptr(), a.dattn.data_ptr(),
                                            a.dqkv.data_ptr(), a.ws_blk.data_ptr() + i * a.ws_bytes, a.ws_bytes)
                             for i in range(m.depth)]
        other = getattr(_HOLDER, "st", None)
        if other is not None and other is not self:
            other.end_hold()
        if L.lib().rgbnm_reduce_hold_begin() != 0:
            L.lib().rgbnm_reduce_hold_cancel()
            L.check(L.lib().rgbnm_reduce_hold_begin(), "reduce_hold_begin")
        self.holding = True
        _HOLDER.st = self

    def end_hold(self):
        if self.holding:
            self.holding = False
            _HOLDER.st = None
            a = self.arena
            L.check(L.lib().rgbnm_reduce_hold_end(a.hold_table.data_ptr(), a.hold_table_host.data_ptr(), a.hold_table.numel(),
                                                  L.stream()), "reduce_hold_end")

    def cancel_hold(self):
        if self.holding:
            self.holding = False
            _HOLDER.st = None
            L.lib().rgbnm_reduce_hold_cancel()

    def __del__(self):
        try:
            self.model._release_arena(self.arena)
        except Exception:
            pass


class _PatchEmbedFn(torch.autograd.Function):
    @staticmethod
    def forward(ctx, y, cbcr, st, w, b, lam=None):
        m, a = st.model, st.arena
        Hb, Wb = y.shape[2], y.shape[3]
        L.check(L.lib().rgbnm_patch_embed_fwd_mix(C.byref(a.cfg), L.dt_of(y.dtype), y.data_ptr(), cbcr.data_ptr(), L.ptr(lam),
                                                  m._conv16.data_ptr(), m._sh_ptr("pe", "ws"), b.data_ptr(),
                                                  m._pos.data_ptr(), a.feat.data_ptr(), a.xbuf(0).data_ptr(), Hb, Wb,
                                                  L.stream()), "patch_embed_fwd")
        ctx.st = st
        st.pe_feat_ok = True
        return a.xbuf(0).detach()

    @staticmethod
    def backward(ctx, dx0):
        st = ctx.st
        m, a = st.model, st.arena
        dx0 = dx0.contiguous()
        gw, gb = m._gview(st.gbuf, "patchembed.projection.0.weight"), m._gview(st.gbuf, "patchembed.projection.0.bias")
        try:
            if getattr(st, "pe_done", None) != dx0.data_ptr():
                L.check(L.lib().rgbnm_patch_embed_bwd(C.byref(a.cfg), dx0.data_ptr(), a.feat.data_ptr(), gw.data_ptr(),
                                                      gb.data_ptr(), a.ws.data_ptr(), a.ws_bytes, L.stream()), "patch_embed_bwd")
        except BaseException:
            st.cancel_hold()
            raise
        st.end_hold()
        if m._grad_sync is not None:
            m._grad_sync.ready(st.gbuf, ["patchembed.projection.0.weight", "patchembed.projection.0.bias"], last=True)
        return None, None, None, gw, gb, None


_PE2_NAMES = ["patchembed.projection_Y.1.weight", "patchembed.projection_Y.1.bias", "patchembed.projection_C.1.weight",
              "patchembed.projection_C.1.bias", "patchembed.linearMix.weight", "patchembed.linearMix.bias"]


class _PatchEmbed2Fn(torch.autograd.Function):

    @staticmethod
    def forward(ctx, y, cbcr, st, wy, by, wc, bc, wm, bm):
        m, a = st.model, st.arena
        lib, dt, M, E = L.lib(), a.cfg.dtype, a.cfg.B * a.cfg.N, a.cfg.E
        Ey = E // 6 * 4
        Hb, Wb = y.shape[2], y.shape[3]
        if (Hb // 2) * (Wb // 2) != a.cfg.N:
            raise ValueError("expected a 28 x 28 block grid")
        es = a.feat.element_size()
        L.check(lib.rgbnm_subblock_embed(L.dt_of(y.dtype), dt, y.data_ptr(), cbcr.data_ptr(), m._conv16.data_ptr(),
                                         a.feat.data_ptr(), a.cfg.B, Hb, Wb, 0, L.stream()), "subblock_embed")
        g, gp = a.pe_g, a.pe_gp
        L.check(lib.rgbnm_gemm_nt(dt, L.EPI_GELU, a.feat.data_ptr(), 384, m._sh_ptr("peY", "ws"), 256, g.data_ptr(), E,
                                  by.data_ptr(), None, 0, gp.data_ptr(), E, None, 0, M, Ey, 256, 0, L.stream()), "pe2 Y")
        L.check(lib.rgbnm_gemm_nt(dt, L.EPI_GELU, a.feat.data_ptr() + 256 * es, 384, m._sh_ptr("peC", "ws"), 128,
                                  g.data_ptr() + Ey * es, E, bc.data_ptr(), None, 0, gp.data_ptr() + Ey * es, E, None,
                                  0, M, E - Ey, 128, 0, L.stream()), "pe2 C")
        L.check(lib.rgbnm_gemm_nt(dt, L.EPI_POS, g.data_ptr(), E, m._sh_ptr("peM", "ws"), E, a.xbuf(0).data_ptr(), E,
                                  bm.data_ptr(), None, 0, None, 0, m._pos.data_ptr(), a.cfg.N, M, E, E, 0, L.stream()),
                "pe2 mix")
        ctx.st = st
        return a.xbuf(0).detach()

    @staticmethod
    def backward(ctx, dx0):
        st = ctx.st
        st.end_hold()
        m, a = st.model, st.arena
        lib, dt, M, E = L.lib(), a.cfg.dtype, a.cfg.B * a.cfg.N, a.cfg.E
        Ey = E // 6 * 4
        dx0 = dx0.contiguous()
        es = a.feat.element_size()
        gr = [m._gview(st.gbuf, n) for n in _PE2_NAMES]
        ws, wsb = a.ws.data_ptr(), a.ws_bytes
        L.check(lib.rgbnm_gemm_tn(dt, dx0.data_ptr(), E, a.pe_g.data_ptr(), E, gr[4].data_ptr(), gr[5].data_ptr(), M, E,
                                  E, 0, 0, ws, wsb, L.stream()), "pe2 dWm")
        dh = a.pe_dh
        L.check(lib.rgbnm_gemm_nt(dt, L.EPI_DGELU, dx0.data_ptr(), E, m._sh_ptr("peM", "wst"), E, dh.data_ptr(), E,
                                  None, a.pe_gp.data_ptr(), E, None, 0, None, 0, M, E, E, 0, L.stream()), "pe2 dh")
        L.check(lib.rgbnm_gemm_tn(dt, dh.data_ptr(), E, a.feat.data_ptr(), 384, gr[0].data_ptr(), gr[1].data_ptr(), M, Ey,
                                  256, 0, 0, ws, wsb, L.stream()), "pe2 dWy")
        L.check(lib.rgbnm_gemm_tn(dt, dh.data_ptr() + Ey * es, E, a.feat.data_ptr() + 256 * es, 384, gr[2].data_ptr(),
                                  gr[3].data_ptr(), M, E - Ey, 128, 0, 0, ws, wsb, L.stream()), "pe2 dWc")
        if m._grad_sync is not None:
            m._grad_sync.ready(st.gbuf, _PE2_NAMES, last=True)
        return (None, None, None) + tuple(gr)


_PES_NAMES = ([f"patchembed.LinearY.{i}.{k}" for i in range(4) for k in ("weight", "bias")] +
              [f"patchembed.LinearC.{i}.{k}" for i in range(2) for k in ("weight", "bias")] +
              ["patchembed.LinearMix.weight", "patchembed.LinearMix.bias"])


class _PatchEmbedSepFn(torch.autograd.Function):

    @staticmethod
    def forward(ctx, y, cbcr, st, *params):
        m, a = st.model, st.arena
        lib, dt, M, E = L.lib(), a.cfg.dtype, a.cfg.B * a.cfg.N, a.cfg.E
        Hb, Wb = y.shape[2], y.shape[3]
        if (Hb // 2) * (Wb // 2) != a.cfg.N:
            raise ValueError("expected a 28 x 28 block grid")
        L.check(lib.rgbnm_subblock_embed(L.dt_of(y.dtype), dt, y.data_ptr(), cbcr.data_ptr(), m._eye16.data_ptr(),
                                         a.feat.data_ptr(), a.cfg.B, Hb, Wb, 0, L.stream()), "subblock_embed")
        wbd, bcat = m._sep_operands(a.cdtype)
        g, gp = a.pe_g, a.pe_gp
        L.check(lib.rgbnm_gemm_nt(dt, L.EPI_GELU, a.feat.data_ptr(), 384, wbd.data_ptr(), 384, g.data_ptr(), E,
                                  bcat.data_ptr(), None, 0, gp.data_ptr(), E, None, 0, M, E, 384, 0, L.stream()), "pe-sep blocks")
        bm = m._named["patchembed.LinearMix.bias"]
        L.check(lib.rgbnm_gemm_nt(dt, L.EPI_POS, g.data_ptr(), E, m._sh_ptr("peMix", "ws"), E, a.xbuf(0).data_ptr(), E,
                                  bm.data_ptr(), None, 0, None, 0, m._pos.data_ptr(), a.cfg.N, M, E, E, 0, L.stream()),
                "pe-sep mix")
        ctx.st = st
        return a.xbuf(0).detach()

    @staticmethod
    def backward(ctx, dx0):
        st = ctx.st
        st.end_hold()
        m, a = st.model, st.arena
        lib, dt, M, E = L.lib(), a.cfg.dtype, a.cfg.B * a.cfg.N, a.cfg.E
        dx0 = dx0.contiguous()
        gr = [m._gview(st.gbuf, n) for n in _PES_NAMES]
        ws, wsb = a.ws.data_ptr(), a.ws_bytes
        L.check(lib.rgbnm_gemm_tn(dt, dx0.data_ptr(), E, a.pe_g.data_ptr(), E, gr[12].data_ptr(), gr[13].data_ptr(), M, E,
                                  E, 0, 0, ws, wsb, L.stream()), "pe-sep dWmix")
        dh = a.pe_dh
        L.check(lib.rgbnm_gemm_nt(dt, L.EPI_DGELU, dx0.data_ptr(), E, m._sh_ptr("peMix", "wst"), E, dh.data_ptr(), E,
                                  None, a.pe_gp.data_ptr(), E, None, 0, None, 0, M, E, E, 0, L.stream()), "pe-sep dh")
        dwbd = torch.empty(E, 384, device=dx0.device, dtype=torch.float32)
        dbcat = torch.empty(E, device=dx0.device, dtype=torch.float32)
        L.check(lib.rgbnm_gemm_tn(dt, dh.data_ptr(), E, a.feat.data_ptr(), 384, dwbd.data_ptr(), dbcat.data_ptr(), M, E,
                                  384, 0, 0, ws, wsb, L.stream()), "pe-sep dWbd")
        e6 = E // 6
        for i in range(6):
            gr[2 * i].copy_(dwbd[i * e6:(i + 1) * e6].index_select(1, m._sep_cols[i]))
            gr[2 * i + 1].copy_(dbcat[i * e6:(i + 1) * e6])
        if m._grad_sync is not None:
            m._grad_sync.ready(st.gbuf, _PES_NAMES, last=True)
        return (None, None, None) + tuple(gr)


_PE3_NAMES = ["patchembed.projectionY.1.weight", "patchembed.projectionY.1.bias", "patchembed.projectionC.1.weight",
              "patchembed.projectionC.1.bias"]


class _PatchEmbedConcatFn(torch.autograd.Function):

    @staticmethod
    def forward(ctx, y, cbcr, st, wy, by, wc, bc):
        m, a = st.model, st.arena
        lib, dt, E, B = L.lib(), a.cfg.dtype, a.cfg.E, a.cfg.B
        if y.shape[2:4] != (28, 28) or cbcr.shape[2:4] != (14, 14):
            raise ValueError("expected a 28 x 28 luma / 14 x 14 chroma block grid")
        idt = L.dt_of(y.dtype)
        zc = m._zero_chroma(2 * B, y.dtype)
        L.check(lib.rgbnm_subblock_embed(idt, dt, y.data_ptr(), cbcr.data_ptr(), m._conv16.data_ptr(), a.feat.data_ptr(),
                                         B, 28, 28, 0, L.stream()), "subblock_embed Y")
        L.check(lib.rgbnm_subblock_embed(idt, dt, cbcr.data_ptr(), zc.data_ptr(), m._conv16.data_ptr(), a.featC.data_ptr(),
                                         2 * B, 14, 14, 0, L.stream()), "subblock_embed C")
        L.check(lib.rgbnm_gemm_nt(dt, L.EPI_POS, a.feat.data_ptr(), 384, m._sh_ptr("peY3", "ws"), 256, a.pe_ty.data_ptr(), E,
                                  by.data_ptr(), None, 0, None, 0, m._pos.data_ptr(), 196, B * 196, E, 256, 0, L.stream()),
                "pe3 Y")
        L.check(lib.rgbnm_gemm_nt(dt, L.EPI_POS, a.featC.data_ptr(), 384, m._sh_ptr("peC3", "ws"), 256, a.pe_tc.data_ptr(), E,
                                  bc.data_ptr(), None, 0, None, 0, m._pos7.data_ptr(), 49, B * 98, E, 256, 0, L.stream()),
                "pe3 C")
        x0 = a.xbuf(0).view(B, 294, E)
        x0[:, :196].copy_(a.pe_ty.view(B, 196, E))
        x0[:, 196:].copy_(a.pe_tc.view(B, 98, E))
        ctx.st = st
        return a.xbuf(0).detach()

    @staticmethod
    def backward(ctx, dx0):
        st = ctx.st
        st.end_hold()
        m, a = st.model, st.arena
        lib, dt, E, B = L.lib(), a.cfg.dtype, a.cfg.E, a.cfg.B
        dxv = dx0.contiguous().view(B, 294, E)
        dty = dxv[:, :196].contiguous()
        dtc = dxv[:, 196:].contiguous()
        gr = [m._gview(st.gbuf, n) for n in _PE3_NAMES]
        ws, wsb = a.ws.data_ptr(), a.ws_bytes
        L.check(lib.rgbnm_gemm_tn(dt, dty.data_ptr(), E, a.feat.data_ptr(), 384, gr[0].data_ptr(), gr[1].data_ptr(),
                                  B * 196, E, 256, 0, 0, ws, wsb, L.stream()), "pe3 dWy")
        L.check(lib.rgbnm_gemm_tn(dt, dtc.data_ptr(), E, a.featC.data_ptr(), 384, gr[2].data_ptr(), gr[3].data_ptr(),
                                  B * 98, E, 256, 0, 0, ws, wsb, L.stream()), "pe3 dWc")
        if m._grad_sync is not None:
            m._grad_sync.ready(st.gbuf, _PE3_NAMES, last=True)
        return (None, None, None) + tuple(gr)


class _BlockFn(torch.autograd.Function):
    @staticmethod
    def forward(ctx, x, st, idx, *params):
        m, a = st.model, st.arena
        assert x.data_ptr() == a.xbuf(idx).data_ptr()
        if st.drop is not None:
            L.check(L.lib().rgbnm_vit_block_fwd_drop(C.byref(a.cfg), C.byref(m._bparams[idx]), C.byref(a.acts[idx]),
                                                     C.byref(st.drop[idx]), L.stream()), "vit_block_fwd_drop")
            ctx.st, ctx.idx = st, idx
            return a.xbuf(idx + 1).detach()
        if idx == 0:
            st.chain_fwd = m._chain_forward(a)
        if st.chain_fwd:
            ctx.st, ctx.idx = st, idx
            return a.xbuf(idx + 1).detach()
        chain = st.ln_chain
        last = idx + 1 >= m.depth
        nxt_p = C.byref(m._bparams[idx + 1]) if chain and not last else None
        nxt_a = C.byref(a.acts[idx + 1]) if chain and not last else None
        L.check(L.lib().rgbnm_vit_block_fwd_chain(C.byref(a.cfg), C.byref(m._bparams[idx]), C.byref(a.acts[idx]),
                                                  1 if (chain and idx > 0) else 0, nxt_p, nxt_a, L.stream()),
                "vit_block_fwd")
        ctx.st, ctx.idx = st, idx
        return a.xbuf(idx + 1).detach()

    @staticmethod
    def backward(ctx, dy):
        st, idx = ctx.st, ctx.idx
        m, a = st.model, st.arena
        dy = dy.contiguous()
        dx = a.dx[idx & 1]
        if dx.data_ptr() == dy.data_ptr():
            dx = a.dx[(idx + 1) & 1]
        grads = [m._gview(st.gbuf, n) for n in m._block_names[idx]]
        g = L.BlockGrads(*[t.data_ptr() for t in grads])
        scratch = a.scratch_blk[idx] if st.holding else a.scratch
        if idx == m.depth - 1:
            m._check_prep_gen(st)
            st.chain_bwd = st.drop is None and m._chain_backward(a, dy)
            st.dw_pending = []
        try:
            if st.drop is not None:
                L.check(L.lib().rgbnm_vit_block_bwd_drop(C.byref(a.cfg), C.byref(m._bparams[idx]), C.byref(a.acts[idx]),
                                                         C.byref(g), C.byref(scratch), C.byref(st.drop[idx]), dy.data_ptr(),
                                                         dx.data_ptr(), L.stream()), "vit_block_bwd_drop")
            elif getattr(st, "chain_bwd", False):
                dx = a.dx_blk[idx]
                st.dw_pending.append((idx, g, dy.data_ptr()))
                if st.gbuf.data_ptr() != m._gflat.data_ptr():
                    group = 1
                elif st.holding:
                    group = m.depth
                elif m._grad_sync is not None:
                    group = m.dw_group_overlapped
                else:
                    group = 1
                if len(st.dw_pending) >= min(group, CHAIN_MAX_DEPTH) or idx == 0:
                    pend, st.dw_pending = st.dw_pending, []
                    n = len(pend)
                    scs = [L.BlockScratch(a.du_blk[i].data_ptr(), a.dxn.data_ptr(), a.dxmid_blk[i].data_ptr(), a.dattn_chain.data_ptr(),
                                          a.dqkv_blk[i].data_ptr(), a.ws_chain.data_ptr() + i * a.ws_bytes, a.ws_bytes)
                           for i, _, _ in pend]
                    pa = (C.POINTER(L.BlockActs) * n)(*[C.pointer(a.acts[i]) for i, _, _ in pend])
                    pg = (C.POINTER(L.BlockGrads) * n)(*[C.pointer(gg) for _, gg, _ in pend])
                    ps = (C.POINTER(L.BlockScratch) * n)(*[C.pointer(x) for x in scs])
                    pdy = (C.c_void_p * n)(*[d for _, _, d in pend])
                    p2 = (C.c_void_p * n)(*[a.lnpart[i, 0].data_ptr() for i, _, _ in pend])
                    p1 = (C.c_void_p * n)(*[a.lnpart[i, 1].data_ptr() for i, _, _ in pend])
                    L.check(L.lib().rgbnm_vit_blocks_bwd_dw(C.byref(a.cfg), n, pa, pg, ps, pdy, p2, p1, L.stream()), "vit_blocks_bwd_dw")
                    if m._grad_sync is not None:
                        for i, _, _ in pend[:-1]:
                            m._grad_sync.ready(st.gbuf, m._block_names[i])
                else:
                    by_name = dict(zip(m._block_names[idx], grads))
                    return (dx, None, None) + tuple(by_name[n] for n in m._block_param_order[idx])
            else:
                L.check(L.lib().rgbnm_vit_block_bwd(C.byref(a.cfg), C.byref(m._bparams[idx]), C.byref(a.acts[idx]),
                                                    C.byref(g), C.byref(scratch), dy.data_ptr(), dx.data_ptr(),
                                                    L.stream()), "vit_block_bwd")
            if m._grad_sync is not None:
                m._grad_sync.ready(st.gbuf, m._block_names[idx])
        except BaseException:
            st.cancel_hold()
            raise
        by_name = dict(zip(m._block_names[idx], grads))
        return (dx, None, None) + tuple(by_name[n] for n in m._block_param_order[idx])


class _EncoderFn(torch.autograd.Function):

    @staticmethod
    def forward(ctx, x, st, *params):
        m, a = st.model, st.arena
        assert x.data_ptr() == a.xbuf(0).data_ptr()
        st.chain_fwd = m._chain_forward(a)
        if not st.chain_fwd:
            chain = st.ln_chain
            for idx in range(m.depth):
                last = idx + 1 >= m.depth
                nxt_p = C.byref(m._bparams[idx + 1]) if chain and not last else None
                nxt_a = C.byref(a.acts[idx + 1]) if chain and not last else None
                L.check(L.lib().rgbnm_vit_block_fwd_chain(C.byref(a.cfg), C.byref(m._bparams[idx]), C.byref(a.acts[idx]),
                                                          1 if (chain and idx > 0) else 0, nxt_p, nxt_a, L.stream()), "vit_block_fwd")
        ctx.st = st
        return a.xbuf(m.depth).detach()

    @staticmethod
    def backward(ctx, dy):
        st = ctx.st
        m, a = st.model, st.arena
        D = m.depth
        dy = dy.contiguous()
        grads = [[m._gview(st.gbuf, n) for n in m._block_names[i]] for i in range(D)]
        gs = [L.BlockGrads(*[t.data_ptr() for t in grads[i]]) for i in range(D)]
        m._check_prep_gen(st)
        try:
            if m._chain_backward(a, dy):
                group = D if (m._grad_sync is None or st.holding) else m.dw_group_overlapped
                group = min(group, CHAIN_MAX_DEPTH)
                idx = D - 1
                while idx >= 0:
                    pend = list(range(idx, max(idx - group, -1), -1))
                    n = len(pend)
                    scs = [L.BlockScratch(a.du_blk[i].data_ptr(), a.dxn.data_ptr(), a.dxmid_blk[i].data_ptr(), a.dattn_chain.data_ptr(),
                                          a.dqkv_blk[i].data_ptr(), a.ws_chain.data_ptr() + i * a.ws_bytes, a.ws_bytes) for i in pend]
                    pa = (C.POINTER(L.BlockActs) * n)(*[C.pointer(a.acts[i]) for i in pend])
                    pg = (C.POINTER(L.BlockGrads) * n)(*[C.pointer(gs[i]) for i in pend])
                    ps = (C.POINTER(L.BlockScratch) * n)(*[C.pointer(x) for x in scs])
                    pdy = (C.c_void_p * n)(*[dy.data_ptr() if i == D - 1 else a.dx_blk[i + 1].data_ptr() for i in pend])
                    p2 = (C.c_void_p * n)(*[a.lnpart[i, 0].data_ptr() for i in pend])
                    p1 = (C.c_void_p * n)(*[a.lnpart[i, 1].data_ptr() for i in pend])
                    pe = None
                    if (pend[-1] == 0 and n == D and m.embed_kind == "group" and getattr(st, "pe_feat_ok", False)
                            and all(p.requires_grad for p in m._pe_params_list())):
                        pe = (m._gview(st.gbuf, "patchembed.projection.0.weight"), m._gview(st.gbuf, "patchembed.projection.0.bias"))
                    if pe is None:
                        L.check(L.lib().rgbnm_vit_blocks_bwd_dw(C.byref(a.cfg), n, pa, pg, ps, pdy, p2, p1, L.stream()), "vit_blocks_bwd_dw")
                    else:
                        L.check(L.lib().rgbnm_vit_blocks_bwd_dw_pe(C.byref(a.cfg), n, pa, pg, ps, pdy, p2, p1, a.dx_blk[0].data_ptr(),
                                                                   a.feat.data_ptr(), pe[0].data_ptr(), pe[1].data_ptr(),
                                                                   a.ws.data_ptr(), a.ws_bytes, L.stream()), "vit_blocks_bwd_dw_pe")
                        st.pe_done = a.dx_blk[0].data_ptr()
                    if m._grad_sync is not None:
                        for i in pend:
                            m._grad_sync.ready(st.gbuf, m._block_names[i])
                    idx -= n
                dx = a.dx_blk[0]
            else:
                cur = dy
                for idx in range(D - 1, -1, -1):
                    dx = a.dx[idx & 1]
                    if dx.data_ptr() == cur.data_ptr():
                        dx = a.dx[(idx + 1) & 1]
                    scratch = a.scratch_blk[idx] if st.holding else a.scratch
                    L.check(L.lib().rgbnm_vit_block_bwd(C.byref(a.cfg), C.byref(m._bparams[idx]), C.byref(a.acts[idx]),
                                                        C.byref(gs[idx]), C.byref(scratch), cur.data_ptr(), dx.data_ptr(),
                                                        L.stream()), "vit_block_bwd")
                    if m._grad_sync is not None:
                        m._grad_sync.ready(st.gbuf, m._block_names[idx])
                    cur = dx
        except BaseException:
            st.cancel_hold()
            raise
        out = []
        for i in range(D):
            by_name = dict(zip(m._block_names[i], grads[i]))
            out += [by_name[n] for n in m._block_param_order[i]]
        return (dx, None) + tuple(out)


class _HeadFn(torch.autograd.Function):
    @staticmethod
    def forward(ctx, x, st, *params):
        m, a = st.model, st.arena
        logits = torch.empty(a.B, m._ncls_pad, device=x.device, dtype=torch.float32)
        acts = L.HeadActs(x.data_ptr(), a.hmean.data_ptr(), a.hrstd.data_ptr(), a.pooled.data_ptr(),
                          a.h1.data_ptr(), logits.data_ptr())
        L.check(L.lib().rgbnm_head_fwd(C.byref(a.cfg), C.byref(m._hparams), C.byref(acts), L.stream()), "head_fwd")
        ctx.st, ctx.acts, ctx.x = st, acts, x
        ctx.set_materialize_grads(False)
        if m._ncls_pad != m.n_classes:
            return logits[:, :m.n_classes].contiguous()
        if a.cdtype == torch.float32:
            return logits
        return logits, torch.empty(a.B, m._ncls_pad, device=x.device, dtype=a.cdtype)

    @staticmethod
    def backward(ctx, dlogits, dedge=None):
        st = ctx.st
        m, a = st.model, st.arena
        if dlogits is None and dedge is None:
            return (None,) * (2 + len(m._head_param_order))
        if dedge is not None:
            dlogits = dedge if dlogits is None else dedge + dlogits.to(dedge.dtype)
        names = m._head_names
        grads = [m._gview(st.gbuf, n) for n in names]
        padded = m._ncls_pad != m.n_classes
        if padded:
            dl = torch.zeros(a.B, m._ncls_pad, device=dlogits.device, dtype=a.cdtype)
            dl[:, :m.n_classes].copy_(dlogits)
            dw2p = torch.empty(m._ncls_pad, m.emb_size, device=dlogits.device, dtype=torch.float32)
            db2p = torch.empty(m._ncls_pad, device=dlogits.device, dtype=torch.float32)
            ptrs = [t.data_ptr() for t in grads]
            ptrs[names.index("classhead.ch_linear2.weight")] = dw2p.data_ptr()
            ptrs[names.index("classhead.ch_linear2.bias")] = db2p.data_ptr()
            g = L.HeadGrads(*ptrs)
        else:
            dl = dlogits.to(a.cdtype).contiguous()
            g = L.HeadGrads(*[t.data_ptr() for t in grads])
        dx = a.dx[0]
        if not padded:
            st.begin_hold()
        ws = a.ws_head if st.holding else a.ws
        try:
            L.check(L.lib().rgbnm_head_bwd(C.byref(a.cfg), C.byref(m._hparams), C.byref(ctx.acts), C.byref(g),
                                           dl.data_ptr(), a.da.data_ptr(), a.dpooled.data_ptr(), dx.data_ptr(),
                                           ws.data_ptr(), ws.numel(), L.stream()), "head_bwd")
            if padded:
                grads[names.index("classhead.ch_linear2.weight")].copy_(dw2p[:m.n_classes])
                grads[names.index("classhead.ch_linear2.bias")].copy_(db2p[:m.n_classes])
            if m._grad_sync is not None:
                m._grad_sync.ready(st.gbuf, names)
        except BaseException:
            st.cancel_hold()
            raise
        if padded:
            st.begin_hold()
        by_name = dict(zip(names, grads))
        return (dx, None) + tuple(by_name[n] for n in m._head_param_order)


class ViT(FlatParamModule):
    defer_grad_reduction = False
    dw_group_overlapped = 4
    single_encoder_node = True
    train_dropout = False
    last_dropout_seed = None

    def __init__(self, in_channels: int = 3, patch_size: int = 16, emb_size: int = 768, input_embed: int = -1,
                 depth: int = 12, n_classes: int = 1000, drop_p=0.1, pixel_space="RGB", ver=1, use_subblock=True,
                 device="cpu", dtype=torch.float32, num_heads: int = 8, head_size: int = 64, **kwargs):
        super().__init__()
        if pixel_space.lower() not in ("dct", "rgb2dct"):
            raise NotImplementedError("rgb-no-more_amd implements the --domain DCT path only")
        if ver not in (1, 2, 3):
            raise NotImplementedError("ver must be 1 (PatchEmbedding_DCT_Group), 2 (PatchEmbedding_DCT_Separate / "
                                      "_Separate_subblock) or 3 (PatchEmbedding_DCT_Concat)")
        if ver in (1, 3) and not use_subblock:
            raise NotImplementedError("embed_type 1 / 3 without sub-block conversion are not in any reference config")
        if not 0.0 <= float(drop_p) < 1.0:
            raise ValueError("dropout probability has to be in [0, 1)")
        self.drop_p = float(drop_p)
        if head_size != 64 or emb_size not in (192, 384, 512, 768, 1024) or input_embed >= 0:
            raise NotImplementedError("HIP kernels cover head_size 64 and emb_size 192 / 384 (JPEG-Ti / JPEG-S; tuned) and "
                                      "512 / 768 / 1024 (vitb / vitl of utils/configs.py:104-122; generic kernels)")
        if dtype != torch.float32:
            raise NotImplementedError("parameters are fp32 masters; choose bf16 compute with autocast")
        if n_classes < 1:
            raise ValueError("n_classes must be positive")
        self.pixel_space = pixel_space
        self.emb_size, self.depth, self.n_classes = emb_size, depth, n_classes
        self._ncls_pad = (n_classes + 7) // 8 * 8
        self.num_heads, self.inner = num_heads, num_heads * head_size
        self.n_tokens = 294 if ver == 3 else 196
        E = emb_size
        kw = dict(device=device, dtype=dtype)
        self.ver = ver
        self.embed_kind = {1: "group", 3: "concat"}.get(ver, "sep_sub" if use_subblock else "sep")
        self.patchembed = {"group": lambda: PatchEmbedding_DCT_Group(patch_size, E, use_subblock, **kw),
                           "sep_sub": lambda: PatchEmbedding_DCT_Separate_subblock(patch_size, E, **kw),
                           "sep": lambda: PatchEmbedding_DCT_Separate(patch_size, E, **kw),
                           "concat": lambda: PatchEmbedding_DCT_Concat(patch_size, E, use_subblock, **kw)}[self.embed_kind]()
        blocks = []
        for _ in range(depth):
            att = ResidualAdd(nn.Sequential(OrderedDict([
                ("eb_lrnorm1", nn.LayerNorm(E, **kw)),
                ("eb_mha", MultiHeadAttention(E, num_heads, head_size, **kw)),
                ("eb_drop1", nn.Identity())])))
            ffn = ResidualAdd(nn.Sequential(OrderedDict([
                ("eb_lrnorm2", nn.LayerNorm(E, **kw)),
                ("eb_ffb", nn.Sequential(nn.Linear(E, 4 * E, **kw), nn.Identity(), nn.Identity(),
                                         nn.Linear(4 * E, E, **kw))),
                ("eb_drop2", nn.Identity())])))
            blocks.append(nn.Sequential(att, ffn))
        self.encoder = nn.Sequential(*blocks)
        self.classhead = nn.Sequential(OrderedDict([
            ("ch_lrnorm", nn.LayerNorm(E, **kw)), ("ch_gap", nn.Identity()),
            ("ch_linear1", nn.Linear(E, E, **kw)), ("ch_tanh", nn.Identity()),
            ("ch_linear2", nn.Linear(E, n_classes, **kw))]))
        self._flat = None
        self._arenas = {}
        self.compute_dtype = None

    def _names(self):
        return [n for n, _ in self.named_parameters()]

    def _flatten(self):
        dev = next(self.parameters()).device
        if dev.type != "cuda":
            raise L.RgbnmError("model parameters must live on a HIP device (no CPU fallback)")
        params = self._pack_parameters()
        offs = self._offs
        if self.embed_kind == "group":
            lin = [("pe", "patchembed.projection.0", 0)]
        elif self.embed_kind == "sep_sub":
            lin = [("peY", "patchembed.projection_Y.1", 0), ("peC", "patchembed.projection_C.1", 0),
                   ("peM", "patchembed.linearMix", 0)]
        elif self.embed_kind == "sep":
            lin = [("peMix", "patchembed.LinearMix", 0)]
        else:
            lin = [("peY3", "patchembed.projectionY.1", 0), ("peC3", "patchembed.projectionC.1", 0)]
        for i in range(self.depth):
            lin += [(f"qkv{i}", f"encoder.{i}.0.fn.eb_mha.qkv", self.num_heads),
                    (f"proj{i}", f"encoder.{i}.0.fn.eb_mha.projection", 0),
                    (f"fc1{i}", f"encoder.{i}.1.fn.eb_ffb.0", 0), (f"fc2{i}", f"encoder.{i}.1.fn.eb_ffb.3", 0)]
        lin += [("h1", "classhead.ch_linear1", 0), ("h2", "classhead.ch_linear2", 0)]
        descs = (L.LinearDesc * len(lin))()
        self._sh_off, so, bo = {}, 0, 0
        chain_ok = self.emb_size == 192 and self.num_heads == 3 and self.n_tokens == 196
        from . import chain as _chain
        kinds = {"eb_mha.qkv": 1, "eb_mha.projection": 2, "eb_ffb.0": 3, "eb_ffb.3": 4}
        for k, (key, name, ph) in enumerate(lin):
            ck = kinds[name.split(".fn.")[1]] if chain_ok and name.startswith("encoder.") else 0
            coff = int(name.split(".")[1]) * _chain.BLOCK_ELEMS if ck else 0
            Nn, Kk = self._shapes[name + ".weight"]
            Np = self._ncls_pad if key == "h2" else Nn
            ws, wst = so, so + _align(Np * Kk)
            so = wst + _align(Np * Kk)
            bp = bo
            if ph:
                bo += _align(Nn)
            descs[k] = L.LinearDesc(offs[name + ".weight"], offs[name + ".bias"], ws, wst, bp, Nn, Kk, ph,
                                    1 if key == "peM" else 0, Np if Np != Nn else 0, 0, ck, coff)
            self._sh_off[key] = (ws, wst, bp)
        self._ndesc, self._sh_total = len(lin), so
        self._descs_dev = torch.frombuffer(bytearray(bytes(descs)), dtype=torch.uint8).to(dev)
        self._bias_perm = torch.zeros(max(bo, 1), device=dev, dtype=torch.float32)
        self._shadow = {}
        if self.embed_kind == "sep":
            self._eye16 = torch.eye(16, device=dev, dtype=torch.float32)
            p1, p2 = torch.meshgrid(torch.arange(8), torch.arange(8), indexing="ij")
            cols = [((pdh * 8 + p1) * 16 + pdw * 8 + p2).reshape(-1) for pdh in range(2) for pdw in range(2)]
            cols += [256 + torch.arange(64), 320 + torch.arange(64)]
            self._sep_cols = [c.to(dev) for c in cols]
            self._sep_cache = {}
        else:
            self._conv16 = self.patchembed.conv_Y.to(dev).contiguous()
        self._chain_idx = None
        self._chain_refused = False
        if chain_ok:
            assert _chain.BLOCK_ELEMS == L.lib().rgbnm_chain_image_elems()
            self._chain_idx = True
            self._chain_img = torch.zeros(self.depth * _chain.BLOCK_ELEMS, device=dev, dtype=torch.bfloat16)
            self._chain_img_bwd = torch.zeros(self.depth * _chain.BLOCK_ELEMS, device=dev, dtype=torch.bfloat16)
        self._pos = sincos_table(14, 14, self.emb_size, dev)
        self._pos7 = sincos_table(7, 7, self.emb_size, dev) if self.embed_kind == "concat" else None
        self._zc = {}
        self._build_names()
        self._arenas = {}
        L.check(L.lib().rgbnm_gelu_table_init(L.stream()), "gelu_table_init")

    def _zero_chroma(self, n, dtype):
        k = (n, dtype)
        if k not in self._zc:
            self._zc[k] = torch.zeros(n, 2, 7, 7, 8, 8, device=self._flat.device, dtype=dtype)
        return self._zc[k]

    def _sep_operands(self, cdtype):
        E, e6 = self.emb_size, self.emb_size // 6
        key = cdtype
        if key not in self._sep_cache:
            self._sep_cache[key] = (torch.zeros(E, 384, device=self._flat.device, dtype=cdtype),
                                    torch.zeros(E, device=self._flat.device, dtype=torch.float32))
        wbd, bcat = self._sep_cache[key]
        named = self._named
        for i in range(6):
            mod = f"patchembed.LinearY.{i}" if i < 4 else f"patchembed.LinearC.{i - 4}"
            wbd[i * e6:(i + 1) * e6].index_copy_(1, self._sep_cols[i], named[mod + ".weight"].detach().to(cdtype))
            bcat[i * e6:(i + 1) * e6].copy_(named[mod + ".bias"].detach())
        return wbd, bcat

    def _build_names(self):
        self._block_names, self._block_param_order, self._bparams_by_dtype = [], [], {}
        for i in range(self.depth):
            a, b = f"encoder.{i}.0.fn.", f"encoder.{i}.1.fn."
            self._block_names.append([a + "eb_lrnorm1.weight", a + "eb_lrnorm1.bias", b + "eb_lrnorm2.weight",
                                      b + "eb_lrnorm2.bias", a + "eb_mha.qkv.weight", a + "eb_mha.qkv.bias",
                                      a + "eb_mha.projection.weight", a + "eb_mha.projection.bias",
                                      b + "eb_ffb.0.weight", b + "eb_ffb.0.bias", b + "eb_ffb.3.weight",
                                      b + "eb_ffb.3.bias"])
            self._block_param_order.append([n for n in self._names() if n.startswith(f"encoder.{i}.")])
        self._head_names = ["classhead.ch_lrnorm.weight", "classhead.ch_lrnorm.bias", "classhead.ch_linear1.weight",
                            "classhead.ch_linear1.bias", "classhead.ch_linear2.weight", "classhead.ch_linear2.bias"]
        self._head_param_order = [n for n in self._names() if n.startswith("classhead.")]
        self._pe_names = {"group": ["patchembed.projection.0.weight", "patchembed.projection.0.bias"], "sep_sub": _PE2_NAMES,
                          "sep": _PES_NAMES, "concat": _PE3_NAMES}[self.embed_kind]

    def grad_ready_order(self):
        if not hasattr(self, "_head_names"):
            self._build_names()
        return ([(self._head_names, False)] + [(self._block_names[i], False) for i in reversed(range(self.depth))] +
                [(self._pe_names, True)])

    def _pe_params_list(self):
        pe = self.__dict__.get("_pe_params")
        if pe is None:
            pe = self.__dict__["_pe_params"] = [p for n, p in self._named.items() if n.startswith("patchembed.")]
        return pe

    def _pptr(self, name):
        return self._flat.data_ptr() + self._offs[name] * 4

    def _sh_ptr(self, key, which):
        sh = self._shadow[self._cur_dtype]
        ws, wst, _ = self._sh_off[key]
        return sh.data_ptr() + (ws if which == "ws" else wst) * sh.element_size()

    def _chain_index_tables(self):
        from . import chain as _chain
        dev = self._flat.device
        idx = np.concatenate([_chain.block_index(self._sh_off[f"qkv{i}"][0], self._sh_off[f"proj{i}"][0],
                                                 self._sh_off[f"fc1{i}"][0], self._sh_off[f"fc2{i}"][0]) for i in range(self.depth)])
        idb = np.concatenate([_chain.block_index_bwd(self._sh_off[f"qkv{i}"][1], self._sh_off[f"proj{i}"][1],
                                                     self._sh_off[f"fc1{i}"][1], self._sh_off[f"fc2{i}"][1])
                              for i in range(self.depth)])
        assert max(idx.max(), idb.max()) < 2 ** 31
        return torch.from_numpy(idx.astype(np.int32)).to(dev), torch.from_numpy(idb.astype(np.int32)).to(dev)

    def _prep(self, cdtype, chains=True):
        if cdtype not in self._shadow:
            self._shadow[cdtype] = torch.zeros(self._sh_total, device=self._flat.device, dtype=cdtype)
        self._cur_dtype = cdtype
        self._prep_gen = getattr(self, "_prep_gen", 0) + 1
        chain = chains and cdtype == torch.bfloat16 and self._chain_idx is not None
        img_f = self._chain_img.data_ptr() if chain and L.lib().rgbnm_get_option(b"fwd_chain") else None
        img_b = (self._chain_img_bwd.data_ptr() if chain and L.lib().rgbnm_get_option(b"bwd_chain") and torch.is_grad_enabled()
                 else None)
        skip = bool(img_f and (img_b or not torch.is_grad_enabled()) and not self._chain_refused)
        L.check(L.lib().rgbnm_prep_weights_chain(L.dt_of(cdtype), self._descs_dev.data_ptr(), self._ndesc, self._flat.data_ptr(),
                                                 self._shadow[cdtype].data_ptr(), self._bias_perm.data_ptr(), img_f, img_b,
                                                 1 if skip else 0, L.stream()), "prep_weights")
        if cdtype not in self._bparams_by_dtype:
            bps = []
            for i in range(self.depth):
                a, b = f"encoder.{i}.0.fn.", f"encoder.{i}.1.fn."
                bps.append(L.BlockParams(
                    self._pptr(a + "eb_lrnorm1.weight"), self._pptr(a + "eb_lrnorm1.bias"),
                    self._pptr(b + "eb_lrnorm2.weight"), self._pptr(b + "eb_lrnorm2.bias"),
                    self._bias_perm.data_ptr() + self._sh_off[f"qkv{i}"][2] * 4,
                    self._pptr(a + "eb_mha.projection.bias"), self._pptr(b + "eb_ffb.0.bias"),
                    self._pptr(b + "eb_ffb.3.bias"),
                    self._sh_ptr(f"qkv{i}", "ws"), self._sh_ptr(f"qkv{i}", "wst"),
                    self._sh_ptr(f"proj{i}", "ws"), self._sh_ptr(f"proj{i}", "wst"),
                    self._sh_ptr(f"fc1{i}", "ws"), self._sh_ptr(f"fc1{i}", "wst"),
                    self._sh_ptr(f"fc2{i}", "ws"), self._sh_ptr(f"fc2{i}", "wst")))
            if self._ncls_pad != self.n_classes and getattr(self, "_b2pad", None) is None:
                self._b2pad = torch.zeros(self._ncls_pad, device=self._flat.device, dtype=torch.float32)
            b2 = self._b2pad.data_ptr() if self._ncls_pad != self.n_classes else self._pptr("classhead.ch_linear2.bias")
            hp = L.HeadParams(self._pptr("classhead.ch_lrnorm.weight"), self._pptr("classhead.ch_lrnorm.bias"),
                              self._pptr("classhead.ch_linear1.bias"), b2,
                              self._sh_ptr("h1", "ws"), self._sh_ptr("h1", "wst"), self._sh_ptr("h2", "ws"),
                              self._sh_ptr("h2", "wst"), self._ncls_pad, 0)
            self._bparams_by_dtype[cdtype] = (bps, hp)
        self._bparams, self._hparams = self._bparams_by_dtype[cdtype]
        if self._ncls_pad != self.n_classes:
            self._b2pad[:self.n_classes].copy_(self._named["classhead.ch_linear2.bias"].detach())

    def _check_prep_gen(self, st):
        if getattr(st, "prep_gen", None) != getattr(self, "_prep_gen", None) and not getattr(self, "_warned_prep_gen", False):
            self._warned_prep_gen = True
            warnings.warn("rgb-no-more_amd: another forward of this model ran between a forward and its backward; the backward uses the "
                          "weight operands of the LATEST forward (identical unless the parameters changed in between)", RuntimeWarning,
                          stacklevel=3)

    def _warn_chain_refused(self, which):
        key = "_warned_chain_" + which
        if not getattr(self, key, False):
            setattr(self, key, True)
            warnings.warn(f"rgb-no-more_amd: the one-launch encoder {which} kernel refused this model (no GELU "
                          f"table); running the per-operation kernels (about 2x slower)", RuntimeWarning, stacklevel=3)

    def _chain_forward(self, a):
        if a.cdtype != torch.bfloat16 or self._chain_idx is None or not L.lib().rgbnm_get_option(b"fwd_chain"):
            return False
        if a.chain_table is None:
            from . import chain as _chain
            blocks = (L.ChainBlock * self.depth)()
            for i in range(self.depth):
                bp, ac = self._bparams[i], a.acts[i]
                blocks[i] = L.ChainBlock(self._chain_img.data_ptr() + i * _chain.BLOCK_ELEMS * 2,
                                         bp.ln1_g, bp.ln1_b, bp.ln2_g, bp.ln2_b, bp.bqkv_perm, bp.bproj, bp.b1, bp.b2,
                                         ac.xn1, ac.mean1, ac.rstd1, ac.qkv, ac.lse, ac.attn, ac.x_mid, ac.xn2, ac.mean2, ac.rstd2,
                                         ac.u, ac.gl, ac.x_out)
            a.chain_table = blocks
        for s0 in range(0, self.depth, CHAIN_MAX_DEPTH):
            n = min(CHAIN_MAX_DEPTH, self.depth - s0)
            sub = C.cast(C.byref(a.chain_table, s0 * C.sizeof(L.ChainBlock)), C.POINTER(L.ChainBlock))
            rc = L.lib().rgbnm_vit_chain_fwd(C.byref(a.cfg), sub, n, a.xbuf(s0).data_ptr(), L.stream())
            if rc == 1 and s0 == 0:
                self._warn_chain_refused("forward")
                if not self._chain_refused:
                    self._chain_refused = True
                    self._prep(a.cdtype)
                return False
            L.check(rc, "vit_chain_fwd")
        return True

    def _chain_backward(self, a, dy):
        if (a.cdtype != torch.bfloat16 or self._chain_idx is None or not a.need_grad
                or not L.lib().rgbnm_get_option(b"bwd_chain")):
            return False
        D, dev = self.depth, self._flat.device
        if a.chain_bwd_table is None or a.chain_bwd_dy != dy.data_ptr():
            from . import chain as _chain
            M, E, I = a.B * self.n_tokens, self.emb_size, self.inner
            if a.chain_bwd_table is None:
                e = lambda *s, dt=a.cdtype: torch.empty(*s, device=dev, dtype=dt)
                a.du_blk = [e(M, 4 * E) for _ in range(D)]
                a.dxmid_blk = [e(M, E) for _ in range(D)]
                a.dqkv_blk = [e(M, 3 * I) for _ in range(D)]
                a.dx_blk = [e(M, E) for _ in range(D)]
                a.dattn_chain = e(M, I)
                a.lnpart = torch.empty(D, 2, a.B, 2, E, device=dev, dtype=torch.float32)
                a.ws_chain = a.ws_blk if a.ws_blk is not None else torch.empty(D * a.ws_bytes, device=dev, dtype=torch.uint8)
            blocks = (L.ChainBwdBlock * D)()
            for i in range(D):
                bp, ac = self._bparams[i], a.acts[i]
                blocks[i] = L.ChainBwdBlock(
                    self._chain_img_bwd.data_ptr() + i * _chain.BLOCK_ELEMS * 2, bp.ln1_g, bp.ln2_g, ac.x_in, ac.mean1, ac.rstd1,
                    ac.qkv, ac.lse, ac.attn, ac.x_mid, ac.mean2, ac.rstd2, ac.u,
                    dy.data_ptr() if i == D - 1 else a.dx_blk[i + 1].data_ptr(),
                    a.du_blk[i].data_ptr(), a.dxmid_blk[i].data_ptr(), a.dqkv_blk[i].data_ptr(), a.dx_blk[i].data_ptr(),
                    a.lnpart[i, 0].data_ptr(), a.lnpart[i, 1].data_ptr())
            a.chain_bwd_table = blocks
            a.chain_bwd_dy = dy.data_ptr()
        starts = list(range(0, D, CHAIN_MAX_DEPTH))
        for s0 in reversed(starts):
            n = min(CHAIN_MAX_DEPTH, D - s0)
            sub = C.cast(C.byref(a.chain_bwd_table, s0 * C.sizeof(L.ChainBwdBlock)), C.POINTER(L.ChainBwdBlock))
            rc = L.lib().rgbnm_vit_chain_bwd(C.byref(a.cfg), sub, n, a.dattn_chain.data_ptr(), L.stream())
            if rc == 1 and s0 == starts[-1]:
                self._warn_chain_refused("backward")
                if not self._chain_refused:
                    self._chain_refused = True
                    self._prep(a.cdtype)
                return False
            L.check(rc, "vit_chain_bwd")
        return True

    def _acquire_arena(self, B, cdtype, need_grad):
        key = (B, cdtype, need_grad)
        pool = self._arenas.setdefault(key, [])
        return pool.pop() if pool else _Arena(self, B, cdtype, need_grad)

    def _release_arena(self, arena):
        pool = self._arenas.setdefault((arena.B, arena.cdtype, arena.need_grad), [])
        if len(pool) < 2:
            pool.append(arena)

    def forward(self, x, cbcr=None):
        if cbcr is None:
            raise ValueError("DCT path needs both Y and CbCr tensors")
        lam = None
        if isinstance(x, LazyMixed) or isinstance(cbcr, LazyMixed):
            if (isinstance(x, LazyMixed) and isinstance(cbcr, LazyMixed) and x.lam.data_ptr() == cbcr.lam.data_ptr()
                    and self.embed_kind == "group"):
                lam, x, cbcr = x.lam, x.tensor, cbcr.tensor
            else:
                x = x.materialize() if isinstance(x, LazyMixed) else x
                cbcr = cbcr.materialize() if isinstance(cbcr, LazyMixed) else cbcr
        L.require_cuda(x, cbcr)
        if x.dim() != 6 or x.shape[1:] != (1, 28, 28, 8, 8) or cbcr.shape[1:] != (2, 14, 14, 8, 8):
            raise ValueError(f"expected Y (B,1,28,28,8,8) and CbCr (B,2,14,14,8,8), got {tuple(x.shape)} {tuple(cbcr.shape)}")
        if x.dtype != cbcr.dtype:
            raise TypeError("Y and CbCr must share a dtype")
        cdtype = self.compute_dtype
        if cdtype is None:
            cdtype = torch.get_autocast_dtype("cuda") if torch.is_autocast_enabled("cuda") else torch.float32
        if cdtype not in (torch.float32, torch.bfloat16, torch.float16):
            raise NotImplementedError(f"compute dtype {cdtype}: the MI355X path implements fp32, bf16 and fp16")
        drop = bool(self.drop_p and self.training)
        if drop and not self.train_dropout:
            raise NotImplementedError("training with dropout p > 0 runs only with model.train_dropout = True (masks from this "
                                      "library's Philox stream, not torch's); model.eval() runs, where nn.Dropout is the identity")
        self._ensure_flat()
        B = x.shape[0]
        need_grad = torch.is_grad_enabled() and any(p.requires_grad for p in self._named.values())
        if need_grad and self._grad_sync is not None:
            self._grad_sync.begin_step()
        self._prep(cdtype, chains=not drop)
        arena = self._acquire_arena(B, cdtype, need_grad)
        st = _FwdState(self, arena, self._grad_buffer() if need_grad else None)
        st.prep_gen = self._prep_gen
        st.ln_chain = bool(L.lib().rgbnm_vit_ln_chain(C.byref(arena.cfg))) and not drop
        if drop:
            self._begin_dropout(st)
        named = self._named
        if self.embed_kind == "group":
            h = _PatchEmbedFn.apply(x, cbcr, st, named["patchembed.projection.0.weight"],
                                    named["patchembed.projection.0.bias"], lam)
        elif self.embed_kind == "sep_sub":
            h = _PatchEmbed2Fn.apply(x, cbcr, st, *[named[n] for n in _PE2_NAMES])
        elif self.embed_kind == "sep":
            h = _PatchEmbedSepFn.apply(x, cbcr, st, *[named[n] for n in _PES_NAMES])
        else:
            h = _PatchEmbedConcatFn.apply(x, cbcr, st, *[named[n] for n in _PE3_NAMES])
        if (not drop and self.single_encoder_node and cdtype == torch.bfloat16 and self._chain_idx is not None
                and L.lib().rgbnm_get_option(b"fwd_chain")):
            h = _EncoderFn.apply(h, st, *self._all_block_params())
        else:
            for i in range(self.depth):
                h = _BlockFn.apply(h, st, i, *[named[n] for n in self._block_param_order[i]])
        out = _HeadFn.apply(h, st, *[named[n] for n in self._head_param_order])
        if isinstance(out, tuple):
            out, edge = out
            out._rgbnm_grad_edge = edge
        return out

    def _begin_dropout(self, st):
        a = st.arena
        st.drop_seed = torch.empty(1, device=self._flat.device, dtype=torch.int64).random_(-2 ** 63, None)
        self.last_dropout_seed = st.drop_seed
        if a.need_grad and getattr(a, "drop_dy", None) is None:
            M, E = a.B * self.n_tokens, self.emb_size
            a.drop_dy = torch.empty(M, E, device=self._flat.device, dtype=a.cdtype)
            a.drop_dxmid = torch.empty(M, E, device=self._flat.device, dtype=a.cdtype)
        dy_m = a.drop_dy.data_ptr() if a.need_grad else None
        dxm_m = a.drop_dxmid.data_ptr() if a.need_grad else None
        st.drop = [L.Dropout(st.drop_seed.data_ptr(), self.drop_p, i, dy_m, dxm_m) for i in range(self.depth)]

    def _all_block_params(self):
        named = self._named
        key = id(named)
        if getattr(self, "_abp_key", None) != key:
            self._abp_key, self._abp = key, [named[n] for i in range(self.depth) for n in self._block_param_order[i]]
        return self._abp
```

Before: 67940.

## Overlap weight prep, head dW flush, and held reduce on side streams; fuse head forward

Adds a per-device side stream with fork/join events. Three pieces of work now run on it in parallel with the main stream: the weight-shadow prep (deferred into the patch-embed forward), the grouped TN flush for the head dW, and the held gradient reduce at the end of the block dW pass. It also adds a fused classifier-head forward kernel that computes fc1+tanh and fc2 in one launch, recomputing h1 per column tile. The aim is to cut serialization and launch gaps in the train step. In exchange it adds stream/event synchronization complexity and redundant h1 work across column tiles.

Result: slower. 66920 (-1.5%).

```diff
diff --git a/include/rgbnm.h b/include/rgbnm.h
--- a/include/rgbnm.h
+++ b/include/rgbnm.h
@@ -258,6 +258,11 @@
                                const rgbnm_block_scratch* const* s, const void* const* dy, const float* const* part2,
                                const float* const* part1, const void* pe_dx0, const void* pe_feat, float* pe_dw, float* pe_db,
                                void* pe_ws, size_t pe_ws_bytes, void* stream);
+int rgbnm_vit_blocks_bwd_dw_pe_hold_end(const rgbnm_vit_cfg* cfg, int n, const rgbnm_block_acts* const* a,
+                                        const rgbnm_block_grads* const* g, const rgbnm_block_scratch* const* s,
+                                        const void* const* dy, const float* const* part2, const float* const* part1,
+                                        const void* pe_dx0, const void* pe_feat, float* pe_dw, float* pe_db, void* pe_ws,
+                                        size_t pe_ws_bytes, void* table, void* table_host, size_t table_bytes, void* stream);
 
 int rgbnm_gelu_table_init(void* stream);
 int rgbnm_gelu_table_info(int* win16, unsigned* full65536);
@@ -273,6 +278,11 @@
 int rgbnm_patch_embed_fwd_mix(const rgbnm_vit_cfg* cfg, int in_dtype, const void* y, const void* cbcr, const float* lam_dev,
                               const float* conv16, const void* wpe, const float* bpe, const float* pos, void* feat, void* x0,
                               int Hb, int Wb, void* stream);
+int rgbnm_patch_embed_fwd_mix_prep(const rgbnm_vit_cfg* cfg, int in_dtype, const void* y, const void* cbcr, const float* lam_dev,
+                                   const float* conv16, const void* wpe, const float* bpe, const float* pos, void* feat, void* x0,
+                                   int Hb, int Wb, const rgbnm_linear_desc* descs_dev, int ndesc, const float* master,
+                                   void* shadow, float* bias_perm, void* chain_fwd, void* chain_bwd, int skip_chain_shadows,
+                                   void* stream);
 int rgbnm_patch_embed_bwd(const rgbnm_vit_cfg* cfg, const void* dx0, const void* feat, float* dwpe, float* dbpe,
                           void* ws, size_t ws_bytes, void* stream);
 
diff --git a/rgb-no-more_amd/csrc/gemm_nt_small.hip b/rgb-no-more_amd/csrc/gemm_nt_small.hip
--- a/rgb-no-more_amd/csrc/gemm_nt_small.hip
+++ b/rgb-no-more_amd/csrc/gemm_nt_small.hip
@@ -82,6 +82,85 @@
     o[e] = (bf16)x;
   }
   *reinterpret_cast<bf16x4*>(reinterpret_cast<bf16*>(p.C) + (size_t)gm * p.ldc + gn) = o;
+}
+
+
+struct HeadFwd {
+  const bf16* pooled; const bf16* W1; const float* b1; bf16* h1; const bf16* W2; const float* b2; float* logits;
+  int M, C, ldc, ntiles;
+};
+
+constexpr int HE = 192, HK = HE / 16, HP = HE + 8;
+
+__global__ __launch_bounds__(256) void head_fwd_fused_kernel(HeadFwd p) {
+  __shared__ __attribute__((aligned(16))) float red[2][4][32 * RP];
+  __shared__ __attribute__((aligned(16))) bf16 h1s[32 * HP];
+  const int tid = threadIdx.x, lane = tid & 63;
+  const int w = __builtin_amdgcn_readfirstlane(tid >> 6);
+  const int l31 = lane & 31, g = lane >> 5;
+  const int ct = blockIdx.x % p.ntiles;
+  const int m0 = (blockIdx.x / p.ntiles) * 32, n0 = ct * 32;
+  const bf16* arow = p.pooled + (size_t)min(m0 + l31, p.M - 1) * HE;
+  const bf16* w2row = p.W2 + (size_t)min(n0 + l31, p.C - 1) * HE;
+  constexpr int PER = HK / 4;
+  Frag<bf16> fa[PER], fw[6][PER], f2[PER];
+#pragma unroll
+  for (int u = 0; u < PER; ++u) fa[u].v = *reinterpret_cast<const bf16x8*>(arow + 16 * (PER * w + u) + 8 * g);
+#pragma unroll
+  for (int t = 0; t < 6; ++t)
+#pragma unroll
+    for (int u = 0; u < PER; ++u)
+      fw[t][u].v = *reinterpret_cast<const bf16x8*>(p.W1 + (size_t)(32 * t + l31) * HE + 16 * (PER * w + u) + 8 * g);
+#pragma unroll
+  for (int u = 0; u < PER; ++u) f2[u].v = *reinterpret_cast<const bf16x8*>(w2row + 16 * (PER * w + u) + 8 * g);
+  const int row = tid >> 3, f0 = (tid & 7) * 4;
+  const int gm = m0 + row;
+#pragma unroll
+  for (int t = 0; t < 6; ++t) {
+    f32x16 acc;
+#pragma unroll
+    for (int r = 0; r < 16; ++r) acc[r] = 0.f;
+#pragma unroll
+    for (int u = 0; u < PER; ++u) mma(acc, fw[t][u], fa[u]);
+#pragma unroll
+    for (int q = 0; q < 4; ++q) {
+      const f32x4 v = {acc[4 * q + 0], acc[4 * q + 1], acc[4 * q + 2], acc[4 * q + 3]};
+      *reinterpret_cast<f32x4*>(&red[t & 1][w][l31 * RP + 8 * q + 4 * g]) = v;
+    }
+    __syncthreads();
+    f32x4 v = *reinterpret_cast<const f32x4*>(&red[t & 1][0][row * RP + f0]);
+#pragma unroll
+    for (int k = 1; k < 4; ++k) v += *reinterpret_cast<const f32x4*>(&red[t & 1][k][row * RP + f0]);
+    v += *reinterpret_cast<const f32x4*>(p.b1 + 32 * t + f0);
+    bf16x4 o;
+#pragma unroll
+    for (int e = 0; e < 4; ++e) o[e] = (bf16)tanhf((float)(bf16)v[e]);
+    *reinterpret_cast<bf16x4*>(&h1s[row * HP + 32 * t + f0]) = o;
+    if (ct == 0 && gm < p.M) *reinterpret_cast<bf16x4*>(p.h1 + (size_t)gm * HE + 32 * t + f0) = o;
+  }
+  __syncthreads();
+  f32x16 acc;
+#pragma unroll
+  for (int r = 0; r < 16; ++r) acc[r] = 0.f;
+#pragma unroll
+  for (int u = 0; u < PER; ++u) {
+    Frag<bf16> fh;
+    fh.v = *reinterpret_cast<const bf16x8*>(&h1s[l31 * HP + 16 * (PER * w + u) + 8 * g]);
+    mma(acc, f2[u], fh);
+  }
+#pragma unroll
+  for (int q = 0; q < 4; ++q) {
+    const f32x4 v = {acc[4 * q + 0], acc[4 * q + 1], acc[4 * q + 2], acc[4 * q + 3]};
+    *reinterpret_cast<f32x4*>(&red[0][w][l31 * RP + 8 * q + 4 * g]) = v;
+  }
+  __syncthreads();
+  const int gn = n0 + f0;
+  if (gm >= p.M || gn >= p.C) return;
+  f32x4 v = *reinterpret_cast<const f32x4*>(&red[0][0][row * RP + f0]);
+#pragma unroll
+  for (int k = 1; k < 4; ++k) v += *reinterpret_cast<const f32x4*>(&red[0][k][row * RP + f0]);
+  if (p.b2) v += *reinterpret_cast<const f32x4*>(p.b2 + gn);
+  *reinterpret_cast<f32x4*>(p.logits + (size_t)gm * p.ldc + gn) = v;
 }
 
 }
@@ -108,3 +187,17 @@
   LAUNCH_CHECK();
   return RGBNM_OK;
 }
+
+int rgbnm_launch_head_fwd_fused(const void* pooled, const void* W1, const float* b1, void* h1, const void* W2, const float* b2,
+                                float* logits, int M, int C, int ldc, hipStream_t st) {
+  if (M < 1 || M > 512 || C < 256 || C % 4 || ldc % 4 || !b1) return 1;
+  HeadFwd p;
+  p.pooled = (const bf16*)pooled; p.W1 = (const bf16*)W1; p.b1 = b1; p.h1 = (bf16*)h1; p.W2 = (const bf16*)W2; p.b2 = b2;
+  p.logits = logits; p.M = M; p.C = C; p.ldc = ldc; p.ntiles = cdiv(C, 32);
+  const double m = M;
+  const int slot = rgbnm_trace_begin(TR_NT, 2.0 * m * HE * (HE + C), (m * HE * 2 + (double)HE * HE + (double)C * HE) * 2.0 + m * C * 4.0, st);
+  hipLaunchKernelGGL(head_fwd_fused_kernel, dim3(cdiv(M, 32) * p.ntiles), dim3(256), 0, st, p);
+  rgbnm_trace_end(slot, st);
+  LAUNCH_CHECK();
+  return RGBNM_OK;
+}
diff --git a/rgb-no-more_amd/csrc/internal.h b/rgb-no-more_amd/csrc/internal.h
--- a/rgb-no-more_amd/csrc/internal.h
+++ b/rgb-no-more_amd/csrc/internal.h
@@ -34,6 +34,8 @@
                          hipStream_t st);
 int rgbnm_launch_nt_small(int epi, const void* A, int lda, const void* W, int ldw, void* C, int ldc, const float* bias,
                           const void* R, int ldr, int c_f32, int M, int N, int K, hipStream_t st);
+int rgbnm_launch_head_fwd_fused(const void* pooled, const void* W1, const float* b1, void* h1, const void* W2, const float* b2,
+                                float* logits, int M, int C, int ldc, hipStream_t st);
 int rgbnm_launch_mlp_bwd(const void* DY, int lddy, const void* W2T, const void* W1T, const void* GP, int ldg, void* DU, int ldu,
                          const void* X, int ldx, const float* gamma, const float* mean, const float* rstd, void* DX, int lddx,
                          float* part, int* npanels_out, int M, int E, int H, hipStream_t st);
@@ -48,5 +50,6 @@
 void rgbnm_reduce_defer_begin();
 int rgbnm_reduce_defer_flush(hipStream_t st);
 int rgbnm_reduce_submit(const RgbnmReduceJob& job, hipStream_t st);
+int rgbnm_reduce_held_count();
 int rgbnm_trace_begin(int tag, double flops, double bytes, hipStream_t st);
 void rgbnm_trace_end(int slot, hipStream_t st);
diff --git a/rgb-no-more_amd/csrc/reduce.hip b/rgb-no-more_amd/csrc/reduce.hip
--- a/rgb-no-more_amd/csrc/reduce.hip
+++ b/rgb-no-more_amd/csrc/reduce.hip
@@ -152,6 +152,8 @@
   return n > 0 ? launch(g_jobs, n, st) : RGBNM_OK;
 }
 
+int rgbnm_reduce_held_count() { return g_hold ? g_held.njobs : -1; }
+
 int rgbnm_reduce_submit(const RgbnmReduceJob& job, hipStream_t st) {
   if (job.n <= 0 || job.S <= 0 || (job.epw != 64 && job.epw != 8)) return RGBNM_EINVAL;
   if (g_hold && g_held.njobs < MAXHELD) {
diff --git a/rgb-no-more_amd/csrc/vit.hip b/rgb-no-more_amd/csrc/vit.hip
--- a/rgb-no-more_amd/csrc/vit.hip
+++ b/rgb-no-more_amd/csrc/vit.hip
@@ -26,7 +26,46 @@
   return e;
 }
 struct Opt { const char* name; std::atomic<int> value; };
-Opt g_opts[] = {{"nt_staged", 1}, {"tn_tr", 1}, {"tn_pipe", 1}, {"attn_v2", 1}, {"nt_wres", 1}, {"nt_kpipe", 1}, {"attn_persist", 1}, {"ln_fuse", 1}, {"tn_group", 2}, {"trace", 0}, {"tn_wgs", 512}, {"mlp_fuse", 1}, {"nt_cold", 0}, {"mlp_bwd", 1}, {"nt_small", 1}, {"mlp_dmast", 1}, {"gelu_table", 1}, {"ln_rows", 1}, {"kp8", 1}, {"win_xcd", 1}, {"kp_persist", 1}, {"fwd_chain", 1}, {"bwd_chain", 1}, {"tn_direct", 1}, {"tn_pack", 1}, {"tn_wide", 1}};
+Opt g_opts[] = {{"nt_staged", 1}, {"tn_tr", 1}, {"tn_pipe", 1}, {"attn_v2", 1}, {"nt_wres", 1}, {"nt_kpipe", 1}, {"attn_persist", 1}, {"ln_fuse", 1}, {"tn_group", 2}, {"trace", 0}, {"tn_wgs", 512}, {"mlp_fuse", 1}, {"nt_cold", 0}, {"mlp_bwd", 1}, {"nt_small", 1}, {"mlp_dmast", 1}, {"gelu_table", 1}, {"ln_rows", 1}, {"kp8", 1}, {"win_xcd", 1}, {"kp_persist", 1}, {"fwd_chain", 1}, {"bwd_chain", 1}, {"tn_direct", 1}, {"tn_pack", 1}, {"tn_wide", 1}, {"branches", 7}, {"branch_forks", 0}, {"head_fuse", 1}};
+
+struct Branch { hipStream_t side = nullptr; hipEvent_t fork = nullptr, join = nullptr; };
+constexpr int BRANCH_DEVS = 16;
+thread_local Branch t_branch[BRANCH_DEVS];
+enum { BR_PREP = 1, BR_HEAD_DW = 2, BR_REDUCE = 4 };
+
+Branch* branch_for(int bit, hipStream_t st) {
+  int on = 0;
+  for (auto& o : g_opts) if (!strcmp(o.name, "branches")) on = o.value.load(std::memory_order_relaxed);
+  if (!(on & bit)) return nullptr;
+  int dev = -1;
+  if (hipGetDevice(&dev) != hipSuccess || dev < 0 || dev >= BRANCH_DEVS) return nullptr;
+  Branch& b = t_branch[dev];
+  if (b.side) return &b;
+  hipStreamCaptureStatus cap = hipStreamCaptureStatusNone;
+  if (hipStreamIsCapturing(st, &cap) != hipSuccess) { (void)hipGetLastError(); return nullptr; }
+  if (cap != hipStreamCaptureStatusNone) return nullptr;
+  Branch nb;
+  if (hipStreamCreateWithFlags(&nb.side, hipStreamNonBlocking) != hipSuccess ||
+      hipEventCreateWithFlags(&nb.fork, hipEventDisableTiming) != hipSuccess ||
+      hipEventCreateWithFlags(&nb.join, hipEventDisableTiming) != hipSuccess) {
+    (void)hipGetLastError();
+    if (nb.join) (void)hipEventDestroy(nb.join);
+    if (nb.fork) (void)hipEventDestroy(nb.fork);
+    if (nb.side) (void)hipStreamDestroy(nb.side);
+    return nullptr;
+  }
+  b = nb;
+  return &b;
+}
+int branch_mark(Branch* b, hipStream_t st) { return hipEventRecord(b->fork, st) == hipSuccess ? RGBNM_OK : RGBNM_ELAUNCH; }
+int branch_enter(Branch* b) {
+  for (auto& o : g_opts) if (!strcmp(o.name, "branch_forks")) o.value.fetch_add(1, std::memory_order_relaxed);
+  return hipStreamWaitEvent(b->side, b->fork, 0) == hipSuccess ? RGBNM_OK : RGBNM_ELAUNCH;
+}
+int branch_join(Branch* b, hipStream_t st) {
+  if (hipEventRecord(b->join, b->side) != hipSuccess) return RGBNM_ELAUNCH;
+  return hipStreamWaitEvent(st, b->join, 0) == hipSuccess ? RGBNM_OK : RGBNM_ELAUNCH;
+}
 }
 
 int rgbnm_trace_begin(int tag, double flops, double bytes, hipStream_t st) {
@@ -315,10 +354,33 @@
   return rgbnm_vit_blocks_bwd_dw_pe(c, n, a, g, s, dy, part2, part1, nullptr, nullptr, nullptr, nullptr, nullptr, 0, st);
 }
 
+struct HoldClose { void* table; void* table_host; size_t table_bytes; };
+static int blocks_bwd_dw(const rgbnm_vit_cfg* c, int n, const rgbnm_block_acts* const* a, const rgbnm_block_grads* const* g,
+                         const rgbnm_block_scratch* const* s, const void* const* dy, const float* const* part2,
+                         const float* const* part1, const void* pe_dx0, const void* pe_feat, float* pe_dw, float* pe_db,
+                         void* pe_ws, size_t pe_ws_bytes, const HoldClose* hc, void* st);
+
 int rgbnm_vit_blocks_bwd_dw_pe(const rgbnm_vit_cfg* c, int n, const rgbnm_block_acts* const* a, const rgbnm_block_grads* const* g,
                                const rgbnm_block_scratch* const* s, const void* const* dy, const float* const* part2,
                                const float* const* part1, const void* pe_dx0, const void* pe_feat, float* pe_dw, float* pe_db,
                                void* pe_ws, size_t pe_ws_bytes, void* st) {
+  return blocks_bwd_dw(c, n, a, g, s, dy, part2, part1, pe_dx0, pe_feat, pe_dw, pe_db, pe_ws, pe_ws_bytes, nullptr, st);
+}
+
+int rgbnm_vit_blocks_bwd_dw_pe_hold_end(const rgbnm_vit_cfg* c, int n, const rgbnm_block_acts* const* a,
+                                        const rgbnm_block_grads* const* g, const rgbnm_block_scratch* const* s,
+                                        const void* const* dy, const float* const* part2, const float* const* part1,
+                                        const void* pe_dx0, const void* pe_feat, float* pe_dw, float* pe_db, void* pe_ws,
+                                        size_t pe_ws_bytes, void* table, void* table_host, size_t table_bytes, void* st) {
+  const HoldClose hc = {table, table_host, table_bytes};
+  return blocks_bwd_dw(c, n, a, g, s, dy, part2, part1, pe_dx0, pe_feat, pe_dw, pe_db, pe_ws, pe_ws_bytes, &hc, st);
+}
+
+static int blocks_bwd_dw(const rgbnm_vit_cfg* c, int n, const rgbnm_block_acts* const* a, const rgbnm_block_grads* const* g,
+                         const rgbnm_block_scratch* const* s, const void* const* dy, const float* const* part2,
+                         const float* const* part1, const void* pe_dx0, const void* pe_feat, float* pe_dw, float* pe_db,
+                         void* pe_ws, size_t pe_ws_bytes, const HoldClose* hc, void* st) {
+  if (hc && rgbnm_reduce_held_count() < 0) hc = nullptr;
   if (!c || n < 1 || n > 12 || !a || !g || !s || !dy || !part2 || !part1) return RGBNM_EINVAL;
   if (pe_dx0 && (!pe_feat || !pe_dw || !pe_ws)) return RGBNM_EINVAL;
   const int dt = c->dtype, M = c->B * c->N, E = c->E, I = c->heads * 64;
@@ -331,7 +393,7 @@
       if (s[k]->ws == s[i]->ws) return RGBNM_EINVAL;
   }
   rgbnm_reduce_defer_begin();
-  bool tn_open = false;
+  bool tn_open = false, side_ok = false;
   const int rc = [&]() -> int {
     const int group = rgbnm_get_option("tn_group");
     if (group) { rgbnm_tn_defer_begin_n(group == 1 ? 2 : 4 * n + (pe_dx0 ? 1 : 0)); tn_open = true; }
@@ -345,7 +407,11 @@
 #undef WS
     }
     if (pe_dx0) TRY(rgbnm_gemm_tn(dt, pe_dx0, E, pe_feat, 384, pe_dw, pe_db, M, E, 384, 0, 0, pe_ws, pe_ws_bytes, st));
+    Branch* br = hc && group ? branch_for(BR_REDUCE, (hipStream_t)st) : nullptr;
+    const int held0 = rgbnm_reduce_held_count();
+    if (br) TRY(branch_mark(br, (hipStream_t)st));
     if (group) { tn_open = false; TRY(rgbnm_tn_defer_flush((hipStream_t)st)); }
+    side_ok = br && rgbnm_reduce_held_count() == held0;
     for (int i = 0; i < n; ++i) {
       RgbnmReduceJob j;
       j.stride = 2LL * E; j.n = E; j.S = c->B; j.cols = 1; j.perm_heads = 0; j.accumulate = 0; j.epw = 8;
@@ -362,7 +428,22 @@
   }();
   const int rt = tn_open ? rgbnm_tn_defer_flush((hipStream_t)st) : RGBNM_OK;
   const int rf = rgbnm_reduce_defer_flush((hipStream_t)st);
-  return rc != RGBNM_OK ? rc : (rt != RGBNM_OK ? rt : rf);
+  int rh = RGBNM_OK;
+  if (hc) {
+    if (rc != RGBNM_OK || rt != RGBNM_OK || rf != RGBNM_OK) {
+      rgbnm_reduce_hold_cancel();
+    } else if (side_ok) {
+      Branch* br = branch_for(BR_REDUCE, (hipStream_t)st);
+      rh = branch_enter(br);
+      if (rh == RGBNM_OK) rh = rgbnm_reduce_hold_end(hc->table, hc->table_host, hc->table_bytes, br->side);
+      else rgbnm_reduce_hold_cancel();
+      const int rj = branch_join(br, (hipStream_t)st);
+      if (rh == RGBNM_OK) rh = rj;
+    } else {
+      rh = rgbnm_reduce_hold_end(hc->table, hc->table_host, hc->table_bytes, st);
+    }
+  }
+  return rc != RGBNM_OK ? rc : (rt != RGBNM_OK ? rt : (rf != RGBNM_OK ? rf : rh));
 }
 
 int rgbnm_vit_block_bwd_dw(const rgbnm_vit_cfg* c, const rgbnm_block_acts* a, const rgbnm_block_grads* g,
@@ -382,6 +463,27 @@
   return RGBNM_OK;
 }
 
+int rgbnm_patch_embed_fwd_mix_prep(const rgbnm_vit_cfg* c, int in_dtype, const void* y, const void* cbcr, const float* lam_dev,
+                                   const float* conv16, const void* wpe, const float* bpe, const float* pos, void* feat, void* x0,
+                                   int Hb, int Wb, const rgbnm_linear_desc* descs_dev, int ndesc, const float* master,
+                                   void* shadow, float* bias_perm, void* chain_fwd, void* chain_bwd, int skip_chain_shadows,
+                                   void* st) {
+  if (!c) return RGBNM_EINVAL;
+  const int M = c->B * c->N;
+  if ((Hb / 2) * (Wb / 2) != c->N) return RGBNM_EINVAL;
+  Branch* br = branch_for(BR_PREP, (hipStream_t)st);
+  if (br) { TRY(branch_mark(br, (hipStream_t)st)); TRY(branch_enter(br)); }
+  const int rp = rgbnm_prep_weights_chain(c->dtype, descs_dev, ndesc, master, shadow, bias_perm, chain_fwd, chain_bwd,
+                                          skip_chain_shadows, br ? (void*)br->side : st);
+  const int rs = rp != RGBNM_OK ? rp : rgbnm_subblock_embed_mix(in_dtype, c->dtype, y, cbcr, lam_dev, conv16, feat, c->B, Hb,
+                                                                Wb, 0, st);
+  if (br) TRY(branch_join(br, (hipStream_t)st));
+  TRY(rs);
+  TRY(rgbnm_gemm_nt(c->dtype, RGBNM_EPI_POS, feat, 384, wpe, 384, x0, c->E, bpe, 0, 0, 0, 0, pos, c->N, M, c->E, 384,
+                    0, st));
+  return RGBNM_OK;
+}
+
 int rgbnm_patch_embed_fwd(const rgbnm_vit_cfg* c, int in_dtype, const void* y, const void* cbcr, const float* conv16,
                           const void* wpe, const float* bpe, const float* pos, void* feat, void* x0, int Hb, int Wb,
                           void* st) {
@@ -398,6 +500,10 @@
   if (!c || !p || !a) return RGBNM_EINVAL;
   const int dt = c->dtype, E = c->E, C = p->n_classes;
   TRY(rgbnm_head_pool_fwd(dt, a->x, p->ln_g, p->ln_b, a->pooled, a->mean, a->rstd, c->B, c->N, E, c->ln_eps, st));
+  if (dt == RGBNM_DT_BF16 && E == 192 && rgbnm_get_option("head_fuse") && rgbnm_get_option("nt_small")) {
+    const int rc = rgbnm_launch_head_fwd_fused(a->pooled, p->w1, p->b1, a->h1, p->w2, p->b2, a->logits, c->B, C, C, (hipStream_t)st);
+    if (rc <= 0) return rc;
+  }
   TRY(rgbnm_gemm_nt(dt, RGBNM_EPI_TANH, a->pooled, E, p->w1, E, a->h1, E, p->b1, 0, 0, 0, 0, 0, 0, c->B, E, E, 0, st));
   TRY(rgbnm_gemm_nt(dt, RGBNM_EPI_NONE, a->h1, E, p->w2, E, a->logits, C, p->b2, 0, 0, 0, 0, 0, 0, c->B, C, E, 1, st));
   return RGBNM_OK;
@@ -429,12 +535,18 @@
     TRY(rgbnm_gemm_tn(dt, da, E, a->pooled, E, g->dw1, g->db1, B, E, E, 0, 0, w2, b2, st));
     return RGBNM_OK;
   }();
-  const int rt = grouped ? rgbnm_tn_defer_flush((hipStream_t)st) : RGBNM_OK;
-  if (rc != RGBNM_OK) return rc;
-  if (rt != RGBNM_OK) return rt;
-  TRY(rgbnm_gemm_nt(dt, RGBNM_EPI_NONE, da, E, p->w1_t, E, dpooled, E, 0, 0, 0, 0, 0, 0, 0, B, E, E, 0, st));
-  TRY(rgbnm_head_pool_bwd(dt, dpooled, a->x, p->ln_g, a->mean, a->rstd, dx, g->dln_g, g->dln_b, B, c->N, E, 0, w3, b3, st));
-  return RGBNM_OK;
-}
-
-}
+  Branch* br = grouped && rc == RGBNM_OK ? branch_for(BR_HEAD_DW, (hipStream_t)st) : nullptr;
+  if (br) { TRY(branch_mark(br, (hipStream_t)st)); TRY(branch_enter(br)); }
+  const int rt = grouped ? rgbnm_tn_defer_flush(br ? br->side : (hipStream_t)st) : RGBNM_OK;
+  const int rd = [&]() -> int {
+    if (rc != RGBNM_OK) return rc;
+    if (rt != RGBNM_OK) return rt;
+    TRY(rgbnm_gemm_nt(dt, RGBNM_EPI_NONE, da, E, p->w1_t, E, dpooled, E, 0, 0, 0, 0, 0, 0, 0, B, E, E, 0, st));
+    TRY(rgbnm_head_pool_bwd(dt, dpooled, a->x, p->ln_g, a->mean, a->rstd, dx, g->dln_g, g->dln_b, B, c->N, E, 0, w3, b3, st));
+    return RGBNM_OK;
+  }();
+  if (br) TRY(branch_join(br, (hipStream_t)st));
+  return rd;
+}
+
+}
diff --git a/rgb-no-more_amd/lib.py b/rgb-no-more_amd/lib.py
--- a/rgb-no-more_amd/lib.py
+++ b/rgb-no-more_amd/lib.py
@@ -165,6 +165,8 @@
     "rgbnm_vit_block_bwd_dw": (_i, [_P(VitCfg), _P(BlockActs), _P(BlockGrads), _P(BlockScratch), _vp, _vp, _vp, _vp]),
     "rgbnm_vit_blocks_bwd_dw": (_i, [_P(VitCfg), _i, _vp, _vp, _vp, _vp, _vp, _vp, _vp]),
     "rgbnm_vit_blocks_bwd_dw_pe": (_i, [_P(VitCfg), _i, _vp, _vp, _vp, _vp, _vp, _vp, _vp, _vp, _vp, _vp, _vp, _sz, _vp]),
+    "rgbnm_vit_blocks_bwd_dw_pe_hold_end": (_i, [_P(VitCfg), _i, _vp, _vp, _vp, _vp, _vp, _vp, _vp, _vp, _vp, _vp, _vp, _sz, _vp, _vp,
+                                                 _sz, _vp]),
     "rgbnm_vit_block_fwd_chain": (_i, [_P(VitCfg), _P(BlockParams), _P(BlockActs), _i, _P(BlockParams), _P(BlockActs), _vp]),
     "rgbnm_vit_block_bwd": (_i, [_P(VitCfg), _P(BlockParams), _P(BlockActs), _P(BlockGrads), _P(BlockScratch), _vp,
                                  _vp, _vp]),
@@ -173,6 +175,8 @@
                                       _vp, _vp, _vp]),
     "rgbnm_patch_embed_fwd": (_i, [_P(VitCfg), _i, _vp, _vp, _vp, _vp, _vp, _vp, _vp, _vp, _i, _i, _vp]),
     "rgbnm_patch_embed_fwd_mix": (_i, [_P(VitCfg), _i, _vp, _vp, _vp, _vp, _vp, _vp, _vp, _vp, _vp, _i, _i, _vp]),
+    "rgbnm_patch_embed_fwd_mix_prep": (_i, [_P(VitCfg), _i, _vp, _vp, _vp, _vp, _vp, _vp, _vp, _vp, _vp, _i, _i, _vp, _i, _vp, _vp,
+                                            _vp, _vp, _vp, _i, _vp]),
     "rgbnm_patch_embed_bwd": (_i, [_P(VitCfg), _vp, _vp, _vp, _vp, _vp, _sz, _vp]),
     "rgbnm_head_fwd": (_i, [_P(VitCfg), _P(HeadParams), _P(HeadActs), _vp]),
     "rgbnm_head_bwd": (_i, [_P(VitCfg), _P(HeadParams), _P(HeadActs), _P(HeadGrads), _vp, _vp, _vp, _vp, _vp, _sz,
diff --git a/rgb-no-more_amd/plainvit.py b/rgb-no-more_amd/plainvit.py
--- a/rgb-no-more_amd/plainvit.py
+++ b/rgb-no-more_amd/plainvit.py
@@ -227,10 +227,17 @@
     def forward(ctx, y, cbcr, st, w, b, lam=None):
         m, a = st.model, st.arena
         Hb, Wb = y.shape[2], y.shape[3]
-        L.check(L.lib().rgbnm_patch_embed_fwd_mix(C.byref(a.cfg), L.dt_of(y.dtype), y.data_ptr(), cbcr.data_ptr(), L.ptr(lam),
-                                                  m._conv16.data_ptr(), m._sh_ptr("pe", "ws"), b.data_ptr(),
-                                                  m._pos.data_ptr(), a.feat.data_ptr(), a.xbuf(0).data_ptr(), Hb, Wb,
-                                                  L.stream()), "patch_embed_fwd")
+        pd = m.__dict__.pop("_prep_deferred", None)
+        if pd is not None:
+            L.check(L.lib().rgbnm_patch_embed_fwd_mix_prep(C.byref(a.cfg), L.dt_of(y.dtype), y.data_ptr(), cbcr.data_ptr(), L.ptr(lam),
+                                                           m._conv16.data_ptr(), m._sh_ptr("pe", "ws"), b.data_ptr(),
+                                                           m._pos.data_ptr(), a.feat.data_ptr(), a.xbuf(0).data_ptr(), Hb, Wb,
+                                                           *pd, L.stream()), "patch_embed_fwd_prep")
+        else:
+            L.check(L.lib().rgbnm_patch_embed_fwd_mix(C.byref(a.cfg), L.dt_of(y.dtype), y.data_ptr(), cbcr.data_ptr(), L.ptr(lam),
+                                                      m._conv16.data_ptr(), m._sh_ptr("pe", "ws"), b.data_ptr(),
+                                                      m._pos.data_ptr(), a.feat.data_ptr(), a.xbuf(0).data_ptr(), Hb, Wb,
+                                                      L.stream()), "patch_embed_fwd")
         ctx.st = st
         st.pe_feat_ok = True
         return a.xbuf(0).detach()
@@ -549,6 +556,14 @@
                         pe = (m._gview(st.gbuf, "patchembed.projection.0.weight"), m._gview(st.gbuf, "patchembed.projection.0.bias"))
                     if pe is None:
                         L.check(L.lib().rgbnm_vit_blocks_bwd_dw(C.byref(a.cfg), n, pa, pg, ps, pdy, p2, p1, L.stream()), "vit_blocks_bwd_dw")
+                    elif st.holding:
+                        L.check(L.lib().rgbnm_vit_blocks_bwd_dw_pe_hold_end(
+                            C.byref(a.cfg), n, pa, pg, ps, pdy, p2, p1, a.dx_blk[0].data_ptr(), a.feat.data_ptr(), pe[0].data_ptr(),
+                            pe[1].data_ptr(), a.ws.data_ptr(), a.ws_bytes, a.hold_table.data_ptr(), a.hold_table_host.data_ptr(),
+                            a.hold_table.numel(), L.stream()), "vit_blocks_bwd_dw_pe_hold_end")
+                        st.holding = False
+                        _HOLDER.st = None
+                        st.pe_done = a.dx_blk[0].data_ptr()
                     else:
                         L.check(L.lib().rgbnm_vit_blocks_bwd_dw_pe(C.byref(a.cfg), n, pa, pg, ps, pdy, p2, p1, a.dx_blk[0].data_ptr(),
                                                                    a.feat.data_ptr(), pe[0].data_ptr(), pe[1].data_ptr(),
@@ -840,7 +855,8 @@
         assert max(idx.max(), idb.max()) < 2 ** 31
         return torch.from_numpy(idx.astype(np.int32)).to(dev), torch.from_numpy(idb.astype(np.int32)).to(dev)
 
-    def _prep(self, cdtype, chains=True):
+    def _prep(self, cdtype, chains=True, defer=False):
+        self._prep_deferred = None
         if cdtype not in self._shadow:
             self._shadow[cdtype] = torch.zeros(self._sh_total, device=self._flat.device, dtype=cdtype)
         self._cur_dtype = cdtype
@@ -850,9 +866,13 @@
         img_b = (self._chain_img_bwd.data_ptr() if chain and L.lib().rgbnm_get_option(b"bwd_chain") and torch.is_grad_enabled()
                  else None)
         skip = bool(img_f and (img_b or not torch.is_grad_enabled()) and not self._chain_refused)
-        L.check(L.lib().rgbnm_prep_weights_chain(L.dt_of(cdtype), self._descs_dev.data_ptr(), self._ndesc, self._flat.data_ptr(),
-                                                 self._shadow[cdtype].data_ptr(), self._bias_perm.data_ptr(), img_f, img_b,
-                                                 1 if skip else 0, L.stream()), "prep_weights")
+        if defer:
+            self._prep_deferred = (self._descs_dev.data_ptr(), self._ndesc, self._flat.data_ptr(), self._shadow[cdtype].data_ptr(),
+                                   self._bias_perm.data_ptr(), img_f, img_b, 1 if skip else 0)
+        else:
+            L.check(L.lib().rgbnm_prep_weights_chain(L.dt_of(cdtype), self._descs_dev.data_ptr(), self._ndesc, self._flat.data_ptr(),
+                                                     self._shadow[cdtype].data_ptr(), self._bias_perm.data_ptr(), img_f, img_b,
+                                                     1 if skip else 0, L.stream()), "prep_weights")
         if cdtype not in self._bparams_by_dtype:
             bps = []
             for i in range(self.depth):
@@ -1001,7 +1021,7 @@
         need_grad = torch.is_grad_enabled() and any(p.requires_grad for p in self._named.values())
         if need_grad and self._grad_sync is not None:
             self._grad_sync.begin_step()
-        self._prep(cdtype, chains=not drop)
+        self._prep(cdtype, chains=not drop, defer=self.embed_kind == "group" and not drop)
         arena = self._acquire_arena(B, cdtype, need_grad)
         st = _FwdState(self, arena, self._grad_buffer() if need_grad else None)
         st.prep_gen = self._prep_gen
```
